# BarisYazici/deep-rl-grasping

Hardware: NVIDIA H100
Metric: SAC grad-steps/sec (batch 256, 64x64 depth) (higher is better)
Workload: dtype bf16x3 (fp32-faithful split, f32 accumulate)

## Files before the change

### deep-rl-grasping_b200/csrc/cg.cu

```cuda
#include <cuda_bf16.h>

#include <cstdio>
#include <cstdlib>

#include "cg.cuh"
#include "common.cuh"
#include "wgmma.cuh"

namespace b2g {
namespace {

constexpr int NMMA_WARPS = 8, NEPI_WARPS = CG_EPI_WARPS, NPROD_WARPS = 2;
constexpr int EPI_WARP0 = NMMA_WARPS, PROD_WARP0 = NMMA_WARPS + NEPI_WARPS;
static_assert(NEPI_WARPS == 4, "the epilogue is one warpgroup: one row of the 128-row tile per lane");
constexpr int NTHREADS = 32 * (PROD_WARP0 + 4);
constexpr int MMA_REGS = 176, EPI_REGS = 136, PROD_REGS = 24;
static_assert(2 * MMA_REGS + EPI_REGS + PROD_REGS <= 512, "register file");
constexpr int STG_BYTES = 2 * 64 * 16 * 4;

__device__ __forceinline__ uint32_t smem_u32(const void* p) { return (uint32_t)__cvta_generic_to_shared(p); }
__device__ __forceinline__ void mbar_init(uint32_t bar, uint32_t count) {
  asm volatile("mbarrier.init.shared::cta.b64 [%0], %1;" ::"r"(bar), "r"(count));
}
__device__ __forceinline__ void mbar_arrive(uint32_t bar) { asm volatile("mbarrier.arrive.shared::cta.b64 _, [%0];" ::"r"(bar) : "memory"); }
__device__ __forceinline__ void mbar_expect_tx(uint32_t bar, uint32_t bytes) {
  asm volatile("mbarrier.arrive.expect_tx.shared::cta.b64 _, [%0], %1;" ::"r"(bar), "r"(bytes) : "memory");
}
__device__ __forceinline__ void mbar_wait(uint32_t bar, uint32_t parity) {
  asm volatile(
      "{\n\t"
      ".reg .pred p;\n\t"
      "CG_WAIT:\n\t"
      "mbarrier.try_wait.parity.shared::cta.b64 p, [%0], %1;\n\t"
      "@p bra CG_DONE;\n\t"
      "bra CG_WAIT;\n\t"
      "CG_DONE:\n\t"
      "}" ::"r"(bar), "r"(parity)
      : "memory");
}
__device__ __forceinline__ bool elect_one() {
  uint32_t pred;
  asm volatile(
      "{\n\t"
      ".reg .pred p;\n\t"
      "elect.sync _|p, 0xffffffff;\n\t"
      "selp.u32 %0, 1, 0, p;\n\t"
      "}"
      : "=r"(pred));
  return pred != 0;
}
__device__ __forceinline__ uint64_t desc_k(uint32_t saddr) { return wg_desc(saddr, 16, 1024); }
__device__ __forceinline__ uint64_t desc_mn(uint32_t saddr, uint32_t lbo) { return wg_desc(saddr, lbo, 1024); }

__device__ __forceinline__ void tma_load(uint32_t dst, const CUtensorMap* map, uint32_t bar, int rank, const int (&c)[5]) {
  switch (rank) {
    case 2:
      asm volatile("cp.async.bulk.tensor.2d.shared::cluster.global.tile.mbarrier::complete_tx::bytes [%0], [%1, {%3, %4}], [%2];" ::"r"(dst), "l"(map),
                   "r"(bar), "r"(c[0]), "r"(c[1])
                   : "memory");
      break;
    case 3:
      asm volatile("cp.async.bulk.tensor.3d.shared::cluster.global.tile.mbarrier::complete_tx::bytes [%0], [%1, {%3, %4, %5}], [%2];" ::"r"(dst),
                   "l"(map), "r"(bar), "r"(c[0]), "r"(c[1]), "r"(c[2])
                   : "memory");
      break;
    case 4:
      asm volatile("cp.async.bulk.tensor.4d.shared::cluster.global.tile.mbarrier::complete_tx::bytes [%0], [%1, {%3, %4, %5, %6}], [%2];" ::"r"(dst),
                   "l"(map), "r"(bar), "r"(c[0]), "r"(c[1]), "r"(c[2]), "r"(c[3])
                   : "memory");
      break;
    default:
      asm volatile("cp.async.bulk.tensor.5d.shared::cluster.global.tile.mbarrier::complete_tx::bytes [%0], [%1, {%3, %4, %5, %6, %7}], [%2];" ::"r"(
                       dst),
                   "l"(map), "r"(bar), "r"(c[0]), "r"(c[1]), "r"(c[2]), "r"(c[3]), "r"(c[4])
                   : "memory");
      break;
  }
}

struct CgPack { CgProblem p[CG_MAX_PROBLEMS]; };
struct Tile { int p, tm, tn, c_begin, c_end; };
struct Walker {
  int p = -1, next_start = 0, tile_start = 0, tiles_n = 1, per = 1, splits = 1, chunks = 0, cps = 0;
  __device__ __forceinline__ bool advance(const CgProblem* __restrict__ probs, int nprob, int tile) {
    bool changed = false;
    while (p < 0 || (p + 1 < nprob && tile >= next_start)) {
      ++p;
      const CgProblem& P = probs[p];
      tile_start = P.tile_start; tiles_n = P.tiles_n; per = P.tiles_m * P.tiles_n; splits = P.splits; chunks = P.chunks;
      cps = (chunks + splits - 1) / splits;
      next_start = p + 1 < nprob ? probs[p + 1].tile_start : 0x7fffffff;
      changed = true;
    }
    return changed;
  }
  __device__ __forceinline__ Tile tile(int t_abs) const {
    int t = t_abs - tile_start, split = 0;
    if (splits > 1) { split = t / per; t -= split * per; }
    Tile ti;
    ti.p = p;
    ti.tm = tiles_n == 1 ? t : t / tiles_n;
    ti.tn = t - ti.tm * tiles_n;
    ti.c_begin = split * cps;
    ti.c_end = min(chunks, ti.c_begin + cps);
    return ti;
  }
};

__device__ __forceinline__ uint32_t pack_bf16x2(float lo, float hi) {
  uint32_t d;
  asm("cvt.rn.bf16x2.f32 %0, %1, %2;" : "=r"(d) : "f"(hi), "f"(lo));
  return d;
}

template <int NT, int NPROD, int TRANS, int KS, int NACC>
__device__ __forceinline__ void mma_chunk(float (&acc)[NACC], uint32_t sbase, uint32_t a_off, uint32_t b_off, uint32_t a_ks, uint32_t b_ks,
                                          uint32_t a_lbo, uint32_t b_lbo, uint32_t a_ps, uint32_t b_ps, uint32_t m_off) {
  constexpr int NPL = NPROD >= 6 ? 3 : (NPROD >= 3 ? 2 : 1), G = NT / 2;
  static_assert(NACC == G * NPL, "one accumulator group of NT columns per product order");
#pragma unroll
  for (int k = 0; k < KS; ++k) {
    uint64_t da[NPL], db[NPL];
#pragma unroll
    for (int pl = 0; pl < NPL; ++pl) {
      const uint32_t pa = sbase + (uint32_t)pl * a_ps + a_off + (uint32_t)k * a_ks + m_off;
      const uint32_t pb = sbase + (uint32_t)pl * b_ps + b_off + (uint32_t)k * b_ks;
      da[pl] = TRANS ? desc_mn(pa, a_lbo) : desc_k(pa);
      db[pl] = TRANS ? desc_mn(pb, b_lbo) : desc_k(pb);
    }
    Wgmma<NT, TRANS>::mma(acc, da[0], db[0]);
    if constexpr (NPL >= 2) Wgmma<NT, TRANS>::mma(acc + G, da[0], db[1]);
    if constexpr (NPL >= 3) Wgmma<NT, TRANS>::mma(acc + 2 * G, da[0], db[2]);
    if constexpr (NPL >= 2) Wgmma<NT, TRANS>::mma(acc + G, da[1], db[0]);
    if constexpr (NPL >= 3) {
      Wgmma<NT, TRANS>::mma(acc + 2 * G, da[1], db[1]);
      Wgmma<NT, TRANS>::mma(acc + 2 * G, da[2], db[0]);
    }
  }
}

__device__ __forceinline__ void mbar_arrive_if(uint32_t bar, bool pred) {
  asm volatile(
      "{\n\t"
      ".reg .pred p;\n\t"
      "setp.ne.u32 p, %1, 0;\n\t"
      "@p mbarrier.arrive.shared::cta.b64 _, [%0];\n\t"
      "}" ::"r"(bar), "r"((uint32_t)pred)
      : "memory");
}
__device__ __forceinline__ void stamp_if(long long* dst, bool pred) {
  asm volatile(
      "{\n\t"
      ".reg .pred p;\n\t"
      ".reg .u64 t;\n\t"
      "mov.u64 t, %%clock64;\n\t"
      "setp.ne.u32 p, %1, 0;\n\t"
      "@p st.global.u64 [%0], t;\n\t"
      "}" ::"l"(dst), "r"((uint32_t)pred)
      : "memory");
}

template <int NT, int NPROD, int TRANS, int KS, class Body>
__device__ __forceinline__ void consume_tile(const CgProblem& P, const Tile& ti, uint32_t ring, uint32_t stg, int slot_bytes, int nstages, uint32_t& s,
                                             uint32_t& ph, uint64_t* bar_full, uint64_t* bar_empty, bool nomma, long long* ctrace, uint32_t& gc,
                                             bool handoff, uint32_t acc_buf, uint32_t& nb, uint64_t* acc_full, uint64_t* acc_empty, Body&& body) {
  constexpr int NGRP = NPROD >= 6 ? 3 : (NPROD >= 3 ? 2 : 1);
  constexpr int NACC = NT / 2 * NGRP;
  const int tid = threadIdx.x, lane = tid & 31, warp = tid >> 5;
  const int wg = warp >> 2, wl = warp & 3, half = wl >> 1;
  float acc[NACC];
#pragma unroll
  for (int j = 0; j < NACC; ++j) acc[j] = 0.f;
  const uint32_t a_ps = (uint32_t)P.a_pstride, b_ps = (uint32_t)P.b_pstride, a_off = P.a_off, b_off = P.b_off, a_ks = P.a_kstep, b_ks = P.b_kstep;
  const uint32_t a_lbo = P.a_lbo, b_lbo = P.b_lbo;
  const uint32_t m_off = TRANS ? (uint32_t)wg * a_lbo : (uint32_t)wg * 8192u;
  uint32_t prev = 0;
  if (nomma) {
    for (int c = ti.c_begin; c < ti.c_end; ++c, ++gc) {
      mbar_wait(smem_u32(&bar_full[s]), (ph >> s) & 1u);
      mbar_arrive_if(smem_u32(&bar_empty[s]), lane == 0);
      ph ^= 1u << s;
      if (++s == (uint32_t)nstages) s = 0;
    }
  } else {
    for (int c = ti.c_begin; c < ti.c_end; ++c, ++gc) {
      long long* const tr = ctrace + gc * 8;
      const bool stamp = ctrace != nullptr && lane == 0 && gc < 64;
      stamp_if(tr + 3, stamp);
      mbar_wait(smem_u32(&bar_full[s]), (ph >> s) & 1u);
      stamp_if(tr + 4, stamp);
      wg_arrive();
      mma_chunk<NT, NPROD, TRANS, KS>(acc, ring + s * (uint32_t)slot_bytes, a_off, b_off, a_ks, b_ks, a_lbo, b_lbo, a_ps, b_ps, m_off);
      wg_commit();
      wg_wait<1>();
      mbar_arrive_if(smem_u32(&bar_empty[prev]), lane == 0 && c > ti.c_begin);
      stamp_if(tr + 5, stamp);
      prev = s;
      ph ^= 1u << s;
      if (++s == (uint32_t)nstages) s = 0;
    }
    wg_wait<0>();
    mbar_arrive_if(smem_u32(&bar_empty[prev]), lane == 0);
  }
  if constexpr (NGRP > 2) {
#pragma unroll
    for (int j = 0; j < NT / 2; ++j) acc[j] = acc[j] + (acc[j + NT / 2] + acc[j + NT]);
  } else if constexpr (NGRP > 1) {
#pragma unroll
    for (int j = 0; j < NT / 2; ++j) acc[j] = acc[j] + acc[j + NT / 2];
  }
  if (handoff) {
    mbar_wait(smem_u32(acc_empty), (nb & 1u) ^ 1u);
    const uint32_t R = 64u * wg + 16u * wl + (uint32_t)(lane >> 2), sw = (uint32_t)(lane >> 2);
    const uint32_t rowa = acc_buf + R * (uint32_t)(NT * 4) + (uint32_t)((lane & 1) * 8);
#pragma unroll
    for (int j = 0; j < NT / 8; ++j)
#pragma unroll
      for (int h = 0; h < 2; ++h) {
        const uint32_t a = rowa + (uint32_t)h * (8u * NT * 4) + ((((uint32_t)(2 * j) + (uint32_t)((lane & 3) >> 1)) ^ sw) << 4);
        asm volatile("st.shared.v2.f32 [%0], {%1,%2};" ::"r"(a), "f"(acc[4 * j + 2 * h]), "f"(acc[4 * j + 2 * h + 1]) : "memory");
      }
    __syncwarp();
    mbar_arrive_if(smem_u32(acc_full), lane == 0);
    ++nb;
    return;
  }
  const int rrow = 32 * (wl & 1) + lane;
  const uint32_t wstg = stg + (uint32_t)wg * 4096u;
#pragma unroll
  for (int R = 0; R < (NT + 63) / 64; ++R) {
    float x[32];
#pragma unroll
    for (int t = 0; t < 4; ++t) {
      const int c0 = 64 * R + 16 * t;
      if (c0 < NT) {
        asm volatile("bar.sync %0, 128;" ::"r"(1 + wg) : "memory");
#pragma unroll
        for (int jj = 0; jj < 2; ++jj)
#pragma unroll
          for (int h = 0; h < 2; ++h) {
            const int row = 16 * wl + (lane >> 2) + 8 * h, chunk = 2 * jj + ((lane & 3) >> 1);
            const int j = c0 / 8 + jj;
            const uint32_t a = wstg + (uint32_t)row * 64u + (uint32_t)((chunk ^ ((row >> 1) & 3)) << 4) + (uint32_t)((lane & 1) * 8);
            asm volatile("st.shared.v2.f32 [%0], {%1,%2};" ::"r"(a), "f"(acc[4 * j + 2 * h]), "f"(acc[4 * j + 2 * h + 1]) : "memory");
          }
        asm volatile("bar.sync %0, 128;" ::"r"(1 + wg) : "memory");
        if (half == (t >> 1)) {
#pragma unroll
          for (int cc = 0; cc < 4; ++cc) {
            const uint32_t a = wstg + (uint32_t)rrow * 64u + (uint32_t)((cc ^ ((rrow >> 1) & 3)) << 4);
            float* xd = x + 16 * (t & 1) + 4 * cc;
            asm volatile("ld.shared.v4.f32 {%0,%1,%2,%3}, [%4];" : "=f"(xd[0]), "=f"(xd[1]), "=f"(xd[2]), "=f"(xd[3]) : "r"(a));
          }
        }
      }
    }
    const int g = 2 * R + half;
    if (32 * g < NT) body(g, x);
  }
}

struct RowOff {
  long long roff = 0, rmoff = 0;
  int ri0 = 0, ri1 = 0;
  __device__ __forceinline__ void set(const CgProblem& Q, int r) {
    const int d0 = Q.d0, d1 = Q.d1;
    const int i0 = r % d0, i12 = r / d0, i1 = i12 % d1, i2 = i12 / d1;
    roff = Q.o_base + (long long)i0 * Q.o0 + (long long)i1 * Q.o1 + (long long)i2 * Q.o2;
    rmoff = Q.m_base + (long long)i0 * Q.m0 + (long long)i1 * Q.m1 + (long long)i2 * Q.m2;
    ri0 = i0; ri1 = i1;
  }
};

__global__ void __launch_bounds__(NTHREADS, 1)
cg_kernel(const __grid_constant__ CgPack pk, int nprob, int total_tiles, const CUtensorMap* __restrict__ maps, int max_stages,
          int dbg, long long* __restrict__ trace) {
  const CgProblem* __restrict__ probs = pk.p;
  extern __shared__ uint8_t smem_raw[];
  __shared__ __align__(8) uint64_t bar_full[CG_MAX_STAGES], bar_empty[CG_MAX_STAGES], acc_full, acc_empty;
  const int tid = threadIdx.x, lane = tid & 31;
  const int warp = __shfl_sync(0xffffffffu, tid >> 5, 0);
  const int trace_cta = dbg >> 8;
  const bool dbg_noload = dbg & 1, dbg_nomma = dbg & 2, dbg_nostore = dbg & 4, dbg_nost = dbg & 16;
  if (tid == 0) {
    for (int s = 0; s < max_stages; ++s) { mbar_init(smem_u32(&bar_full[s]), 1); mbar_init(smem_u32(&bar_empty[s]), NMMA_WARPS); }
    mbar_init(smem_u32(&acc_full), NMMA_WARPS);
    mbar_init(smem_u32(&acc_empty), NEPI_WARPS);
    asm volatile("fence.mbarrier_init.release.cluster;" ::: "memory");
  }
  __syncthreads();
  const uint32_t stg = (smem_u32(smem_raw) + 1023u) & ~1023u;
  const uint32_t ring = stg + STG_BYTES;
  pdl_trigger();
  pdl_wait();

  if (warp >= PROD_WARP0) {
    asm volatile("setmaxnreg.dec.sync.aligned.u32 %0;" ::"n"(PROD_REGS));
    const int pw = warp - PROD_WARP0;
    if (pw >= NPROD_WARPS) return;
    {
      uint32_t gc = 0, s = 0, ph = 0, nbuf = 0;
      int slot_bytes = 0, nstages = 1;
      bool handoff = false;
      Walker w;
      int n2 = 1, nloads = 0, planes = 0, tx = 0;
      const int* tab = nullptr;
      for (int tile = blockIdx.x; tile < total_tiles; tile += gridDim.x) {
        if (w.advance(probs, nprob, tile)) {
          const CgProblem& P = probs[w.p];
          n2 = P.n2; nloads = P.nloads; planes = P.planes; tx = P.tx_bytes; tab = P.tm_tab; handoff = cg_epi_handoff(P.epi);
          if (P.slot_bytes != slot_bytes || P.nstages != nstages) {
            for (int q = 0; q < nstages; ++q) mbar_wait(smem_u32(&bar_empty[q]), ((ph >> q) & 1u) ^ 1u);
            if (nbuf) {
              mbar_wait(smem_u32(&acc_full), (nbuf - 1) & 1u);
              mbar_wait(smem_u32(&acc_empty), (nbuf - 1) & 1u);
              asm volatile("fence.proxy.async.shared::cta;" ::: "memory");
            }
            slot_bytes = P.slot_bytes; nstages = P.nstages; s = 0;
          }
        }
        const Tile ti = w.tile(tile);
        const CgProblem& P = probs[ti.p];
        if (handoff && ti.c_end > ti.c_begin) ++nbuf;
        if (P.dep_ctr) {
          const int* __restrict__ ctr = P.dep_ctr;
          const int x0 = P.dep_by_chunk ? ti.c_begin : ti.tm, x1 = P.dep_by_chunk ? ti.c_end : ti.tm + 1;
          const int lo = x0 * P.dep_rows / P.dep_rows_tile, hi = min(P.dep_tiles - 1, (x1 * P.dep_rows - 1) / P.dep_rows_tile);
          const int expect = P.dep_expect * NEPI_WARPS;
          for (int j = lo + lane; j <= hi; j += 32) {
            int seen;
            do {
              asm volatile("ld.acquire.gpu.global.s32 %0, [%1];" : "=r"(seen) : "l"(ctr + j) : "memory");
              if (seen < expect) __nanosleep(100);
            } while (seen < expect);
          }
          __syncwarp();
          asm volatile("fence.proxy.async.global;" ::: "memory");
        }
        int base[CG_MAX_LOADS][5];
#pragma unroll
        for (int l = 0; l < CG_MAX_LOADS; ++l) {
          if (l < nloads) {
            const CgLoad& L = P.ld[l];
#pragma unroll
            for (int d = 0; d < 5; ++d) base[l][d] = L.c0[d] + ti.tm * L.d_tm[d] + ti.tn * L.d_tn[d];
            if (tab) { base[l][1] += tab[(ti.tm * CG_MAX_LOADS + l) * 2]; base[l][2] += tab[(ti.tm * CG_MAX_LOADS + l) * 2 + 1]; }
          }
        }
        int c1 = n2 > 1 ? ti.c_begin / n2 : 0, c2 = ti.c_begin - c1 * n2;
        for (int c = ti.c_begin; c < ti.c_end; ++c, ++gc) {
          const bool tr = trace && blockIdx.x == trace_cta && pw == 0 && gc < 64 && lane == 0;
          if (tr) trace[gc * 8 + 0] = clock64();
          mbar_wait(smem_u32(&bar_empty[s]), ((ph >> s) & 1u) ^ 1u);
          if (tr) trace[gc * 8 + 1] = clock64();
          const uint32_t full = smem_u32(&bar_full[s]);
          const bool leader = elect_one();
          if (dbg_noload) { if (pw == 0 && leader) mbar_arrive(full); }
          else {
            if (pw == 0 && leader) mbar_expect_tx(full, (uint32_t)tx);
            const uint32_t sbase = ring + s * (uint32_t)slot_bytes;
            int j = 0;
#pragma unroll
            for (int l = 0; l < CG_MAX_LOADS; ++l) {
              if (l < nloads) {
                const CgLoad& L = P.ld[l];
                int crd[5];
#pragma unroll
                for (int d = 0; d < 5; ++d) crd[d] = base[l][d] + c1 * L.d_c1[d] + c2 * L.d_c2[d];
                if (L.plane_box) {
                  if ((j & (NPROD_WARPS - 1)) == pw && leader) tma_load(sbase + (uint32_t)L.smem_off, maps + L.map, full, L.rank, crd);
                  ++j;
                } else {
                  for (int pl = 0; pl < planes; ++pl, ++j) {
#pragma unroll
                    for (int d = 2; d < 5; ++d) if (d == L.rank - 1) crd[d] = pl;
                    if ((j & (NPROD_WARPS - 1)) == pw && leader)
                      tma_load(sbase + (uint32_t)(pl * L.plane_stride + L.smem_off), maps + L.map, full, L.rank, crd);
                  }
                }
              }
            }
          }
          if (tr) { trace[gc * 8 + 2] = clock64(); trace[gc * 8 + 6] = ti.p * 100000 + ti.tm * 10 + ti.tn; }
          if (++c2 == n2) { c2 = 0; ++c1; }
          ph ^= 1u << s;
          if (++s == (uint32_t)nstages) s = 0;
        }
      }
    }
  } else if (warp < NMMA_WARPS) {
    asm volatile("setmaxnreg.inc.sync.aligned.u32 %0;" ::"n"(MMA_REGS));
    const int q = 2 * (warp >> 2) + (warp & 1);
    uint32_t it = 0, s = 0, ph = 0, gc = 0, nb = 0;
    int slot_bytes = 0, nstages = 1;
    Walker w;
    long long* const ctrace = trace && blockIdx.x == trace_cta && warp == 0 ? trace : nullptr;
    const int r = q * 32 + lane;
    int epi = 0, rows_tile = 0, lim_rows = 0, umma_n = 0, n_valid = 0, shape = 0;
    bool handoff = false;
    uint32_t acc_buf = 0;
    long long o_tm = 0;
    RowOff ro;
    for (int tile = blockIdx.x; tile < total_tiles; tile += gridDim.x) {
      if (w.advance(probs, nprob, tile)) {
        const CgProblem& Q = probs[w.p];
        epi = Q.epi; rows_tile = Q.rows_tile; lim_rows = Q.lim_rows; umma_n = Q.umma_n; n_valid = Q.n_valid; o_tm = Q.o_tm;
        ro.set(Q, r);
        shape = cg_shape_key(Q.umma_n, Q.nprod, Q.mn_major != 0, Q.ksteps);
        if (Q.slot_bytes != slot_bytes || Q.nstages != nstages) { slot_bytes = Q.slot_bytes; nstages = Q.nstages; s = 0; }
        handoff = cg_epi_handoff(epi);
        acc_buf = ring + (uint32_t)(nstages * slot_bytes);
      }
      const Tile ti = w.tile(tile);
      if (ti.c_end <= ti.c_begin) continue;
      const CgProblem& P = probs[ti.p];
      const bool valid0 = r < rows_tile && ti.tm * rows_tile + r < lim_rows;
      const long long off0 = ro.roff + (long long)ti.tm * o_tm;
      const int n0 = ti.tn * umma_n;
      const bool tre = trace && blockIdx.x == trace_cta && warp == 0 && lane == 0 && it < 16;
      if (tre) trace[512 + it * 4 + 0] = clock64();
      auto body = [&](int g, float (&x)[32]) {
        const int ng = n0 + 32 * g;
        if (dbg_nostore || ng >= n_valid || !valid0) return;
        float* dst = P.out_f + off0 + (long long)(ng >> 5) * P.f_grp;
        if (epi == CG_EPI_RAW) {
          if (P.atomic) {
#pragma unroll
            for (int j = 0; j < 8; ++j)
              asm volatile("red.global.add.v4.f32 [%0], {%1,%2,%3,%4};" ::"l"(dst + 4 * j), "f"(x[4 * j]), "f"(x[4 * j + 1]), "f"(x[4 * j + 2]),
                           "f"(x[4 * j + 3])
                           : "memory");
          } else {
#pragma unroll
            for (int j = 0; j < 8; ++j) *reinterpret_cast<float4*>(dst + 4 * j) = make_float4(x[4 * j], x[4 * j + 1], x[4 * j + 2], x[4 * j + 3]);
          }
          return;
        }
        const float sc = P.scale;
        if (P.atomic) {
#pragma unroll
          for (int j = 0; j < 8; ++j)
            asm volatile("red.global.add.v4.f32 [%0], {%1,%2,%3,%4};" ::"l"(dst + 4 * j), "f"(x[4 * j] * sc), "f"(x[4 * j + 1] * sc),
                         "f"(x[4 * j + 2] * sc), "f"(x[4 * j + 3] * sc)
                         : "memory");
        } else {
#pragma unroll
          for (int j = 0; j < 8; ++j)
            *reinterpret_cast<float4*>(dst + 4 * j) = make_float4(x[4 * j] * sc, x[4 * j + 1] * sc, x[4 * j + 2] * sc, x[4 * j + 3] * sc);
          if (P.dp_n > 1) {
            const int i4 = (int)((dst - P.dp_gbase) >> 2), per4 = P.dp_per4;
#pragma unroll
            for (int j = 0; j < 8; ++j) {
              const int owner = (i4 + j) / per4;
              if (owner != P.dp_rank)
                reinterpret_cast<float4*>(P.dp_recv[owner])[(size_t)P.dp_rank * per4 + (i4 + j - owner * per4)] =
                    make_float4(x[4 * j] * sc, x[4 * j + 1] * sc, x[4 * j + 2] * sc, x[4 * j + 3] * sc);
            }
          }
        }
      };
#define CG_CONSUME(NT, NPROD, TRANS, KS)                                                                                                      \
  consume_tile<NT, NPROD, TRANS, KS>(P, ti, ring, stg, slot_bytes, nstages, s, ph, bar_full, bar_empty, dbg_nomma, ctrace, gc, handoff, acc_buf, \
                                     nb, &acc_full, &acc_empty, body)
      switch (shape) {
        case cg_shape_key(32, 6, false, 4): CG_CONSUME(32, 6, 0, 4); break;
        case cg_shape_key(64, 6, false, 4): CG_CONSUME(64, 6, 0, 4); break;
        case cg_shape_key(64, 3, false, 4): CG_CONSUME(64, 3, 0, 4); break;
        case cg_shape_key(128, 3, false, 4): CG_CONSUME(128, 3, 0, 4); break;
        case cg_shape_key(64, 3, true, 4): CG_CONSUME(64, 3, 1, 4); break;
        case cg_shape_key(64, 3, true, 9): CG_CONSUME(64, 3, 1, 9); break;
        case cg_shape_key(128, 3, true, 4): CG_CONSUME(128, 3, 1, 4); break;
        default: __trap();
      }
#undef CG_CONSUME
      if (tre) {
        trace[512 + it * 4 + 1] = clock64();
        trace[512 + it * 4 + 2] = handoff;
        trace[512 + it * 4 + 3] = ti.p * 100000 + ti.tm * 10 + ti.tn;
      }
      ++it;
    }
  } else {
    asm volatile("setmaxnreg.inc.sync.aligned.u32 %0;" ::"n"(EPI_REGS));
    const int ew = warp - EPI_WARP0;
    const int r = ew * 32 + lane;
    uint32_t ne = 0;
    int slot_bytes = 0, nstages = 1;
    Walker w;
    int epi = 0, rows_tile = 0, lim_rows = 0, umma_n = 0, out_planes = 0, grp_stride = 32, n_valid = 0, grp_tab = 0;
    bool handoff = false;
    uint32_t acc_buf = 0;
    long long o_tm = 0, m_tm = 0;
    RowOff ro;
    const float* __restrict__ bias = nullptr;
    const uint16_t* __restrict__ mask = nullptr;
    for (int tile = blockIdx.x; tile < total_tiles; tile += gridDim.x) {
      if (w.advance(probs, nprob, tile)) {
        const CgProblem& Q = probs[w.p];
        epi = Q.epi; rows_tile = Q.rows_tile; lim_rows = Q.lim_rows; umma_n = Q.umma_n; out_planes = Q.out_planes;
        grp_stride = Q.grp_stride; n_valid = Q.n_valid; o_tm = Q.o_tm; m_tm = Q.m_tm; bias = Q.bias; mask = Q.mask; grp_tab = Q.grp_tab;
        ro.set(Q, r);
        if (Q.slot_bytes != slot_bytes || Q.nstages != nstages) { slot_bytes = Q.slot_bytes; nstages = Q.nstages; }
        handoff = cg_epi_handoff(epi);
        acc_buf = ring + (uint32_t)(nstages * slot_bytes);
      }
      const Tile ti = w.tile(tile);
      if (ti.c_end <= ti.c_begin || !handoff) continue;
      const CgProblem& P = probs[ti.p];
      const bool valid0 = r < rows_tile && ti.tm * rows_tile + r < lim_rows;
      const long long off0 = ro.roff + (long long)ti.tm * o_tm, moff0 = ro.rmoff + (long long)ti.tm * m_tm;
      const int n0 = ti.tn * umma_n, ngroups = umma_n >> 5;
      auto group_at = [&](int g, bool& valid, long long& off, long long& moff) {
        const int ng = n0 + 32 * g;
        valid = valid0; off = off0; moff = moff0;
        if (grp_tab) {
          const int gg = ng >> 5;
          valid = valid0 && ro.ri0 < P.grp_lim0[gg] && ro.ri1 < P.grp_lim1[gg];
          off = off0 + P.grp_off[gg]; moff = moff0 + P.grp_moff[gg] - ng;
        }
      };
      const bool tre = trace && blockIdx.x == trace_cta && ew == 0 && lane == 0 && ne < 16;
      if (tre) trace[576 + ne * 4 + 0] = clock64();
      uint32_t mbits[4] = {0u, 0u, 0u, 0u};
      if (epi == CG_EPI_DGRAD && !dbg_nostore) {
#pragma unroll
        for (int g = 0; g < 4; ++g) {
          bool valid;
          long long off, moff;
          group_at(g, valid, off, moff);
          const int ng = n0 + 32 * g;
          if (g < ngroups && valid && ng < n_valid) {
            uint4 mk[4];
#pragma unroll
            for (int j = 0; j < 4; ++j) mk[j] = __ldg(reinterpret_cast<const uint4*>(mask + moff + ng) + j);
#pragma unroll
            for (int j = 0; j < 4; ++j) {
              const uint32_t wd[4] = {mk[j].x, mk[j].y, mk[j].z, mk[j].w};
#pragma unroll
              for (int uu = 0; uu < 4; ++uu) {
                if (wd[uu] & 0x00007FFFu) mbits[g] |= 1u << (8 * j + 2 * uu);
                if (wd[uu] & 0x7FFF0000u) mbits[g] |= 1u << (8 * j + 2 * uu + 1);
              }
            }
          }
        }
      }
      mbar_wait(smem_u32(&acc_full), ne & 1u);
      if (tre) trace[576 + ne * 4 + 1] = clock64();
      const bool split_fin = P.ws != nullptr;
      float* __restrict__ wsrow = split_fin ? P.ws + ((size_t)(ti.tm * w.tiles_n + ti.tn) * 128 + r) * umma_n : nullptr;
      auto body = [&](int g, float (&x)[32], int pass) {
        const int ng = n0 + 32 * g;
        bool valid;
        long long off, moff;
        group_at(g, valid, off, moff);
        if (pass == 0 && split_fin) {
#pragma unroll
          for (int j = 0; j < 8; ++j)
            asm volatile("red.global.add.v4.f32 [%0], {%1,%2,%3,%4};" ::"l"(wsrow + 32 * g + 4 * j), "f"(x[4 * j]), "f"(x[4 * j + 1]), "f"(x[4 * j + 2]),
                         "f"(x[4 * j + 3])
                         : "memory");
          return;
        }
        const bool live = !dbg_nostore && ng < n_valid;
        float4 bv[8];
        if (epi == CG_EPI_ACT && live) {
#pragma unroll
          for (int j = 0; j < 8; ++j) bv[j] = __ldg(reinterpret_cast<const float4*>(bias + (long long)(ng >> 5) * P.bias_grp) + j);
        }
        if (!live) return;
        if (epi == CG_EPI_ACT) {
#pragma unroll
          for (int j = 0; j < 8; ++j) {
            x[4 * j] = fmaxf(x[4 * j] + bv[j].x, 0.f); x[4 * j + 1] = fmaxf(x[4 * j + 1] + bv[j].y, 0.f);
            x[4 * j + 2] = fmaxf(x[4 * j + 2] + bv[j].z, 0.f); x[4 * j + 3] = fmaxf(x[4 * j + 3] + bv[j].w, 0.f);
          }
          if (P.f0 > 0 && valid && !dbg_nost) {
            float* dst = P.out_f + (long long)ti.tm * P.f_tm + (long long)r * P.f0 + (long long)(ng >> 5) * P.f_grp;
#pragma unroll
            for (int j = 0; j < 8; ++j) *reinterpret_cast<float4*>(dst + 4 * j) = make_float4(x[4 * j], x[4 * j + 1], x[4 * j + 2], x[4 * j + 3]);
          }
        } else {
          const uint32_t mb = g == 0 ? mbits[0] : g == 1 ? mbits[1] : g == 2 ? mbits[2] : mbits[3];
#pragma unroll
          for (int j = 0; j < 32; ++j)
            if (!((mb >> j) & 1u)) x[j] = 0.f;
          if (P.colsum) {
            float cs[32];
#pragma unroll
            for (int j = 0; j < 32; ++j) cs[j] = x[j];
#pragma unroll
            for (int wd = 16; wd >= 1; wd >>= 1) {
              const bool up = (lane & wd) != 0;
#pragma unroll
              for (int j = 0; j < wd; ++j) {
                const float send = up ? cs[j] : cs[j + wd], keep = up ? cs[j + wd] : cs[j];
                cs[j] = keep + __shfl_xor_sync(0xffffffffu, send, wd);
              }
            }
            atomicAdd(P.colsum + ((ng + lane) & P.colsum_mask), cs[0]);
          }
        }
        const long long gcol = grp_tab ? 0 : (long long)(ng >> 5) * grp_stride;
#pragma unroll 1
        for (int pl = 0; pl < out_planes; ++pl) {
          uint32_t pk[16];
#pragma unroll
          for (int j = 0; j < 16; ++j) {
            pk[j] = pack_bf16x2(x[2 * j], x[2 * j + 1]);
            x[2 * j] -= __uint_as_float(pk[j] << 16);
            x[2 * j + 1] -= __uint_as_float(pk[j] & 0xFFFF0000u);
          }
          if (valid && !dbg_nost) {
            uint16_t* dst = P.out_p[pl] + off + gcol;
#pragma unroll
            for (int j = 0; j < 4; ++j) *reinterpret_cast<uint4*>(dst + 8 * j) = make_uint4(pk[4 * j], pk[4 * j + 1], pk[4 * j + 2], pk[4 * j + 3]);
          }
        }
      };
      const uint32_t rowa = acc_buf + (uint32_t)(r * umma_n * 4), sw = (uint32_t)(r & 7);
      for (int g = 0; g < ngroups; ++g) {
        float x[32];
#pragma unroll
        for (int cc = 0; cc < 8; ++cc) {
          const uint32_t a = rowa + ((((uint32_t)(8 * g + cc)) ^ sw) << 4);
          asm volatile("ld.shared.v4.f32 {%0,%1,%2,%3}, [%4];" : "=f"(x[4 * cc]), "=f"(x[4 * cc + 1]), "=f"(x[4 * cc + 2]), "=f"(x[4 * cc + 3]) : "r"(a));
        }
        if (g == ngroups - 1) {
          __syncwarp();
          mbar_arrive_if(smem_u32(&acc_empty), lane == 0);
        }
        body(g, x, 0);
      }
      ++ne;
      bool last_arriver = !split_fin;
      if (split_fin) {
        __syncwarp();
        int old = 0;
        if (lane == 0) { __threadfence(); old = atomicAdd(P.ws_cnt + (ti.tm * w.tiles_n + ti.tn) * NEPI_WARPS + ew, 1); }
        old = __shfl_sync(0xffffffffu, old, 0);
        last_arriver = old == w.splits - 1;
        if (last_arriver) {
          __threadfence();
          if (lane == 0) P.ws_cnt[(ti.tm * w.tiles_n + ti.tn) * NEPI_WARPS + ew] = 0;
          for (int g = 0; g < ngroups; ++g) {
            float x[32];
#pragma unroll
            for (int j = 0; j < 8; ++j) {
              const float4 sum = __ldcg(reinterpret_cast<const float4*>(wsrow + 32 * g) + j);
              x[4 * j] = sum.x; x[4 * j + 1] = sum.y; x[4 * j + 2] = sum.z; x[4 * j + 3] = sum.w;
              __stcg(reinterpret_cast<float4*>(wsrow + 32 * g) + j, make_float4(0.f, 0.f, 0.f, 0.f));
            }
            body(g, x, 1);
          }
        }
      }
      __syncwarp();
      if (lane == 0 && P.done_ctr && last_arriver) {
        __threadfence();
        atomicAdd(P.done_ctr + ti.tm, 1);
      }
      if (tre) { trace[576 + (ne - 1) * 4 + 2] = clock64(); trace[576 + (ne - 1) * 4 + 3] = ti.p * 100000 + ti.tm * 10 + ti.tn; }
    }
  }
}

typedef CUresult (*EncodeTiledFn)(CUtensorMap*, CUtensorMapDataType, cuuint32_t, void*, const cuuint64_t*, const cuuint64_t*, const cuuint32_t*,
                                  const cuuint32_t*, CUtensorMapInterleave, CUtensorMapSwizzle, CUtensorMapL2promotion, CUtensorMapFloatOOBfill);
EncodeTiledFn g_encode = nullptr;

}

bool cg_shape_supported(int umma_n, int nprod, bool mn_major, int ksteps) {
  switch (cg_shape_key(umma_n, nprod, mn_major, ksteps)) {
    case cg_shape_key(32, 6, false, 4): case cg_shape_key(64, 6, false, 4): case cg_shape_key(64, 3, false, 4): case cg_shape_key(128, 3, false, 4):
    case cg_shape_key(64, 3, true, 4): case cg_shape_key(64, 3, true, 9): case cg_shape_key(128, 3, true, 4): return true;
    default: return false;
  }
}

int cg_smem_limit() { return 226 * 1024 - STG_BYTES; }

int cg_encode_map(CUtensorMap* out, const void* base, int rank, const uint64_t* dims, const uint64_t* strides_bytes, const uint32_t* box,
                  const uint32_t* elem_strides) {
  if (!g_encode) {
    cudaDriverEntryPointQueryResult q;
    void* fn = nullptr;
    if (cudaGetDriverEntryPoint("cuTensorMapEncodeTiled", &fn, cudaEnableDefault, &q) != cudaSuccess || !fn || q != cudaDriverEntryPointSuccess) return -1;
    g_encode = (EncodeTiledFn)fn;
  }
  cuuint64_t gd[5], gs[5];
  cuuint32_t bx[5], es[5];
  for (int i = 0; i < rank; ++i) { gd[i] = dims[i]; bx[i] = box[i]; es[i] = elem_strides ? elem_strides[i] : 1; }
  for (int i = 0; i + 1 < rank; ++i) gs[i] = strides_bytes[i];
  const CUresult r = g_encode(out, CU_TENSOR_MAP_DATA_TYPE_BFLOAT16, (cuuint32_t)rank, const_cast<void*>(base), gd, gs, bx, es, CU_TENSOR_MAP_INTERLEAVE_NONE,
                              CU_TENSOR_MAP_SWIZZLE_128B, CU_TENSOR_MAP_L2_PROMOTION_L2_256B, CU_TENSOR_MAP_FLOAT_OOB_FILL_NONE);
  return r == CUDA_SUCCESS ? 0 : (int)r;
}

int cg_finalize(CgGroup& g, int smem_budget) {
  int start = 0, slot = 0;
  g.flops = 0;
  for (int i = 0; i < g.n; ++i) {
    CgProblem& P = g.host[i];
    P.tile_start = start;
    start += P.tiles_m * P.tiles_n * P.splits;
    for (int l = 0; l < P.nloads; ++l) {
      CgLoad& L = P.ld[l];
      L.plane_stride = L.smem_off >= P.b_off ? P.b_pstride : P.a_pstride;
      if (L.plane_box && L.box_bytes != L.plane_stride) return -2;
    }
    const int need = P.b_off + P.planes * P.b_pstride;
    P.slot_bytes = (need + 1023) / 1024 * 1024;
    slot = slot > P.slot_bytes ? slot : P.slot_bytes;
  }
  g.total_tiles = start;
  const int avail = smem_budget - 1024 ;
  g.slot_bytes = slot; g.nstages = 0;
  int ring = 0;
  for (int i = 0; i < g.n; ++i) {
    CgProblem& P = g.host[i];
    const int acc = cg_epi_handoff(P.epi) ? cg_acc_bytes(P.umma_n) : 0;
    const int avail_ring = avail - acc;
    P.nstages = P.slot_bytes > 0 ? avail_ring / P.slot_bytes : 0;
    if (P.nstages > CG_MAX_STAGES) P.nstages = CG_MAX_STAGES;
    if (P.nstages < 2) return -1;
    P.slot_bytes = avail_ring / P.nstages / 1024 * 1024;
    g.nstages = g.nstages > P.nstages ? g.nstages : P.nstages;
    ring = ring > P.nstages * P.slot_bytes + acc ? ring : P.nstages * P.slot_bytes + acc;
  }
  g.ring_bytes = ring;
  return 0;
}

long long* g_cg_trace = nullptr;

cudaError_t cg_launch(const CgGroup& g, const CUtensorMap* dev_maps, int num_sms, cudaStream_t s, bool pdl, int debug_flags) {
  if (g.total_tiles <= 0 || (debug_flags & 8)) return cudaSuccess;
  static bool attr_set = false;
  if (!attr_set) {
    cudaError_t e = cudaFuncSetAttribute(cg_kernel, cudaFuncAttributeMaxDynamicSharedMemorySize, 226 * 1024);
    if (e != cudaSuccess) return e;
    attr_set = true;
  }
  const int smem = 1024 + STG_BYTES + g.ring_bytes;
  const int grid = g.total_tiles < num_sms ? g.total_tiles : num_sms;
  CgPack pk;
  static_assert(sizeof(CgPack) < 28 * 1024, "problem list must fit the kernel parameter space (32,764 B)");
  for (int i = 0; i < g.n; ++i) pk.p[i] = g.host[i];
  cudaError_t e = launch_pdl(cg_kernel, dim3(grid), dim3(NTHREADS), (size_t)smem, s, pdl, pk, g.n, g.total_tiles, dev_maps, g.nstages, debug_flags, g_cg_trace);
  if (e != cudaSuccess) fprintf(stderr, "cg_launch %s: %s (grid %d, %d threads, smem %d)\n", g.name, cudaGetErrorString(e), grid, NTHREADS, smem);
  return e;
}

}
```

### deep-rl-grasping_b200/csrc/cg.cuh

```cuda
#pragma once
#include <cuda.h>
#include <cuda_runtime.h>
#include <stdint.h>

namespace b2g {

constexpr int CG_MAX_LOADS = 4;
constexpr int CG_MAX_PROBLEMS = 16;
constexpr int CG_MAX_STAGES = 8;
constexpr int CG_MAX_PLANES = 3;
constexpr int CG_EPI_WARPS = 4;

enum CgEpiKind : int {
  CG_EPI_ACT = 0,
  CG_EPI_RAW = 1,
  CG_EPI_DGRAD = 2,
  CG_EPI_WGRAD = 3,
};
__host__ __device__ constexpr bool cg_epi_handoff(int epi) { return epi == CG_EPI_ACT || epi == CG_EPI_DGRAD; }
__host__ __device__ constexpr int cg_acc_bytes(int umma_n) { return 128 * umma_n * 4; }

struct CgLoad {
  int map;
  int rank;
  int box_bytes;
  int smem_off;
  int plane_stride;
  int plane_box;
  int c0[5];
  int d_tm[5], d_tn[5], d_c1[5], d_c2[5];
};

struct CgProblem {
  int tile_start, tiles_m, tiles_n, splits;
  int chunks, n2;
  int nloads, planes;
  int a_pstride, b_pstride;
  int tx_bytes;
  int slot_bytes, nstages;
  CgLoad ld[CG_MAX_LOADS];
  const int* tm_tab;
  int mn_major;
  int ksteps;
  int a_off, b_off;
  int a_kstep, b_kstep;
  int a_lbo, b_lbo;
  int umma_n;
  int nprod;
  int epi;
  int rows_tile;
  int lim_rows;
  int d0, d1;
  long long o_tm; int o0, o1, o2; long long o_base;
  long long m_tm; int m0, m1, m2; long long m_base;
  int n_valid;
  int grp_stride;
  int grp_tab;
  int grp_off[8], grp_moff[8], grp_lim0[8], grp_lim1[8];
  int out_planes;
  uint16_t* out_p[CG_MAX_PLANES];
  float* out_f;
  long long f_tm; int f0;
  const float* bias;
  int bias_grp;
  long long f_grp;
  const uint16_t* mask;
  float* colsum;
  int colsum_mask;
  int atomic;
  float scale;
  int* done_ctr;
  const int* dep_ctr;
  int dep_rows, dep_rows_tile, dep_tiles, dep_expect;
  float* ws;
  int* ws_cnt;
  float* dp_recv[8];
  const float* dp_gbase;
  int dp_rank, dp_n, dp_per4;
  int dep_by_chunk;
};

struct CgGroup {
  CgProblem host[CG_MAX_PROBLEMS];
  int n = 0;
  int total_tiles = 0;
  int slot_bytes = 0, nstages = 0, ring_bytes = 0;
  const char* name = "";
  double flops = 0;
};

int cg_encode_map(CUtensorMap* out, const void* base, int rank, const uint64_t* dims, const uint64_t* strides_bytes, const uint32_t* box,
                  const uint32_t* elem_strides);
int cg_finalize(CgGroup& g, int smem_budget);
cudaError_t cg_launch(const CgGroup& g, const CUtensorMap* dev_maps, int num_sms, cudaStream_t s, bool pdl, int debug_flags);
int cg_smem_limit();
__host__ __device__ constexpr int cg_shape_key(int umma_n, int nprod, bool mn_major, int ksteps) {
  return ksteps * 8192 + umma_n * 16 + nprod * 2 + (mn_major ? 1 : 0);
}
bool cg_shape_supported(int umma_n, int nprod, bool mn_major, int ksteps);

}
```

### deep-rl-grasping_b200/csrc/engine_v2.cu

```cuda
#include <cuda_bf16.h>

#include <algorithm>
#include <cstdio>
#include <cstdlib>
#include <cstring>

#include "sac_internal.cuh"

namespace b2g {
namespace {

struct Gather2Args {
  GatherArgs g;
  uint16_t* a1[2][3];
  uint16_t* fp[3][3];
  int KF, Ci, OH, OW;
};

__device__ __forceinline__ void split3(float y, uint16_t& p0, uint16_t& p1, uint16_t& p2) {
  const __nv_bfloat16 h0 = __float2bfloat16_rn(y);
  const float r1 = y - __bfloat162float(h0);
  const __nv_bfloat16 h1 = __float2bfloat16_rn(r1);
  const float r2 = r1 - __bfloat162float(h1);
  p0 = __bfloat16_as_ushort(h0); p1 = __bfloat16_as_ushort(h1); p2 = __bfloat16_as_ushort(__float2bfloat16_rn(r2));
}

__global__ void __launch_bounds__(512) gather2_kernel(Gather2Args a) {
  extern __shared__ uint16_t sm_planes[];
  const GatherArgs& g = a.g;
  const int b = blockIdx.x, which = blockIdx.y, tid = threadIdx.x;
  const int Ci = a.Ci, HW = g.H * g.W, npx = HW * Ci;
  const int Ec = npx + 4;
  long long slot = b;
  if (g.indices) slot = g.indices[b];
  else if (g.rng_counters) {
    slot = philox_slot(g.seed, (unsigned long long)g.rng_counters[4], b, (unsigned long long)g.rng_counters[5]);
    if (g.ring_cap > 0) slot = ring_slot(g.rng_counters[6], (int)slot, g.ring_cap);
    if (g.indices_out && which == 0 && tid == 0) g.indices_out[b] = (int)slot;
  }
  const unsigned char* __restrict__ src =
      g.obs_frame ? g.frames + (size_t)(which ? g.next_frame : g.obs_frame)[slot] * g.frame_bytes
                  : reinterpret_cast<const unsigned char*>((which ? g.next_obs : g.obs) + (size_t)slot * Ec);
  const double clip_obs = g.normc[1];
  const bool norm_obs = g.normc[3] != 0.0;
  const float scale = g.scale;
  const int rowe = g.W * Ci, pitch = rowe + 8, plane_e = g.H * pitch;
  for (int e4 = tid; e4 < (npx >> 2); e4 += blockDim.x) {
    const float4 v = frame_load4(src, g.fmt, npx, Ci, 4 * e4);
    float y[4] = {v.x, v.y, v.z, v.w};
    if (norm_obs) {
      const double2 m0 = *reinterpret_cast<const double2*>(g.mean + 4 * e4), m1 = *reinterpret_cast<const double2*>(g.mean + 4 * e4 + 2);
      const double2 i0 = *reinterpret_cast<const double2*>(g.var + 4 * e4), i1 = *reinterpret_cast<const double2*>(g.var + 4 * e4 + 2);
      y[0] = (float)fmin(fmax(((double)y[0] - m0.x) * i0.x, -clip_obs), clip_obs);
      y[1] = (float)fmin(fmax(((double)y[1] - m0.y) * i0.y, -clip_obs), clip_obs);
      y[2] = (float)fmin(fmax(((double)y[2] - m1.x) * i1.x, -clip_obs), clip_obs);
      y[3] = (float)fmin(fmax(((double)y[3] - m1.y) * i1.y, -clip_obs), clip_obs);
    }
    uint16_t p[3][4];
#pragma unroll
    for (int j = 0; j < 4; ++j) split3(y[j] / scale, p[0][j], p[1][j], p[2][j]);
#pragma unroll
    for (int pl = 0; pl < 3; ++pl) {
      const uint2 w = make_uint2((uint32_t)p[pl][0] | ((uint32_t)p[pl][1] << 16), (uint32_t)p[pl][2] | ((uint32_t)p[pl][3] << 16));
      const int e = 4 * e4, row = e / rowe, col = e - row * rowe;
      *reinterpret_cast<uint2*>(sm_planes + pl * plane_e + row * pitch + col) = w;
    }
  }
  if (tid == 0) {
    float yy = frame_elem(src, g.fmt, npx, Ci, npx);
    if (norm_obs) yy = (float)fmin(fmax(((double)yy - g.mean[npx]) * g.var[npx], -clip_obs), clip_obs);
    yy = yy / scale;
    uint16_t p0, p1, p2;
    split3(yy, p0, p1, p2);
    const size_t fo = (size_t)b * g.FS + g.feat_col, po = (size_t)b * a.KF + g.feat_col;
    if (which) { g.F_t[fo] = yy; a.fp[2][0][po] = p0; a.fp[2][1][po] = p1; a.fp[2][2][po] = p2; }
    else {
      g.F_pi[fo] = yy; g.F_v[fo] = yy;
      a.fp[0][0][po] = p0; a.fp[0][1][po] = p1; a.fp[0][2][po] = p2;
      a.fp[1][0][po] = p0; a.fp[1][1][po] = p1; a.fp[1][2][po] = p2;
    }
  }
  __syncthreads();
  const int seg = 8 * Ci;
  const int K1 = 64 * Ci, nruns = a.OH * a.OW * 8;
  const size_t img = (size_t)b * a.OH * a.OW * K1;
  for (int i = tid; i < nruns * (seg / 8); i += blockDim.x) {
    const int part = i % (seg / 8), run = i / (seg / 8);
    const int ky = run & 7, patch = run >> 3;
    const int oy = patch / a.OW, ox = patch - oy * a.OW;
    const int so = (4 * oy + ky) * pitch + 4 * ox * Ci + 8 * part;
    const size_t go = img + (size_t)patch * K1 + ky * seg + 8 * part;
#pragma unroll
    for (int pl = 0; pl < 3; ++pl) {
      const uint16_t* sp = sm_planes + pl * plane_e + so;
      const uint2 lo = *reinterpret_cast<const uint2*>(sp), hi = *reinterpret_cast<const uint2*>(sp + 4);
      *reinterpret_cast<uint4*>(a.a1[which][pl] + go) = make_uint4(lo.x, lo.y, hi.x, hi.y);
    }
  }
  if (which == 0 && g.act) {
    const int feat_dim = g.feat_col + 1;
    if (tid < g.n_act) {
      const float av = g.act[slot * g.n_act + tid];
      g.F_v[(size_t)b * g.FS + feat_dim + tid] = av;
      uint16_t p0, p1, p2;
      split3(av, p0, p1, p2);
      const size_t po = (size_t)b * a.KF + feat_dim + tid;
      a.fp[1][0][po] = p0; a.fp[1][1][po] = p1; a.fp[1][2][po] = p2;
    }
    if (tid == 32) {
      float r = g.rew[slot];
      if (g.normc[4] != 0.0) r = (float)fmin(fmax((double)r * g.normc[0], -g.normc[2]), g.normc[2]);
      g.rew_out[b] = r;
      g.done_out[b] = g.done[slot];
    }
  }
}

struct Plane2Job {
  const float* src;
  uint16_t* dst[3];
  int R, N, np;
  int transpose;
  int ld, off0;
  int tile_start;
};

__global__ void __launch_bounds__(256) planes2_kernel(const Plane2Job* __restrict__ jobs, const int* __restrict__ cta_job) {
  __shared__ float tile[64][33];
  const Plane2Job job = jobs[cta_job[blockIdx.x]];
  const int t = blockIdx.x - job.tile_start;
  const int tiles_n = (job.N + 31) / 32;
  const int r0 = (t / tiles_n) * 64, n0 = (t % tiles_n) * 32;
  const int tid = threadIdx.x;
  const bool vec_ok = (job.N & 3) == 0;
  for (int i = tid; i < 64 * 8; i += 256) {
    const int rr = i >> 3, c4 = i & 7, r = r0 + rr, n = n0 + 4 * c4;
    float4 v = make_float4(0.f, 0.f, 0.f, 0.f);
    if (r < job.R) {
      const float* sp = job.src + (size_t)r * job.N + n;
      if (vec_ok && n + 3 < job.N) v = *reinterpret_cast<const float4*>(sp);
      else { if (n < job.N) v.x = sp[0]; if (n + 1 < job.N) v.y = sp[1]; if (n + 2 < job.N) v.z = sp[2]; if (n + 3 < job.N) v.w = sp[3]; }
    }
    tile[rr][4 * c4] = v.x; tile[rr][4 * c4 + 1] = v.y; tile[rr][4 * c4 + 2] = v.z; tile[rr][4 * c4 + 3] = v.w;
    if (!job.transpose && r < job.R) {
      const float x[4] = {v.x, v.y, v.z, v.w};
      uint16_t p[3][4];
#pragma unroll
      for (int u = 0; u < 4; ++u) split3(x[u], p[0][u], p[1][u], p[2][u]);
      for (int k = 0; k < job.np; ++k) {
        uint16_t* d = job.dst[k] + (size_t)r * job.ld + job.off0 + n;
        if (n + 3 < job.N && (((size_t)r * job.ld + job.off0 + n) & 3) == 0)
          *reinterpret_cast<uint2*>(d) = make_uint2((uint32_t)p[k][0] | ((uint32_t)p[k][1] << 16), (uint32_t)p[k][2] | ((uint32_t)p[k][3] << 16));
        else
          for (int u = 0; u < 4; ++u) if (n + u < job.N) d[u] = p[k][u];
      }
    }
  }
  if (!job.transpose) return;
  __syncthreads();
  {
    const int nn = tid >> 3, g8 = tid & 7, n = n0 + nn, rb = r0 + 8 * g8;
    if (n < job.N && rb < job.R) {
      uint16_t p[3][8];
#pragma unroll
      for (int u = 0; u < 8; ++u) split3(tile[8 * g8 + u][nn], p[0][u], p[1][u], p[2][u]);
      const size_t o = (size_t)(n + job.off0) * job.ld + rb;
      for (int k = 0; k < job.np; ++k) {
        uint16_t* d = job.dst[k] + o;
        if (rb + 7 < job.R && (o & 7) == 0)
          *reinterpret_cast<uint4*>(d) = make_uint4((uint32_t)p[k][0] | ((uint32_t)p[k][1] << 16), (uint32_t)p[k][2] | ((uint32_t)p[k][3] << 16),
                                                    (uint32_t)p[k][4] | ((uint32_t)p[k][5] << 16), (uint32_t)p[k][6] | ((uint32_t)p[k][7] << 16));
        else
          for (int u = 0; u < 8; ++u) if (rb + u < job.R) d[u] = p[k][u];
      }
    }
  }
}

int add_maps(V2State& v, uint16_t* const* planes, int np, int rank, std::initializer_list<uint64_t> dims, std::initializer_list<uint64_t> strides_b,
             std::initializer_list<uint32_t> box, std::initializer_list<uint32_t> estr = {}, bool allow_whole = true) {
  uint64_t d[5] = {1, 1, 1, 1, 1}, s[5] = {0, 0, 0, 0, 0};
  uint32_t bx[5] = {1, 1, 1, 1, 1}, es[5] = {1, 1, 1, 1, 1};
  int i = 0; for (auto x : dims) d[i++] = x;
  i = 0; for (auto x : strides_b) s[i++] = x;
  i = 0; for (auto x : box) bx[i++] = x;
  i = 0; for (auto x : estr) es[i++] = x;
  if (rank >= 5 || np < 1) return -1;
  size_t rows = 1;
  for (int k = 1; k < rank; ++k) rows *= (bx[k] + es[k] - 1) / es[k];
  const size_t box_bytes = rows * bx[0] * 2;
  const bool whole = allow_whole && np > 1 && box_bytes % 1024 == 0;
  const long long pitch = np > 1 ? (long long)((const char*)planes[1] - (const char*)planes[0]) : 16;
  for (int p = 2; p < np; ++p)
    if ((const char*)planes[p] - (const char*)planes[p - 1] != pitch) return -1;
  if (pitch <= 0 || pitch % 16) return -1;
  d[rank] = (uint64_t)np; s[rank - 1] = (uint64_t)pitch; bx[rank] = whole ? (uint32_t)np : 1u; es[rank] = 1;
  CUtensorMap m;
  if (cg_encode_map(&m, planes[0], rank + 1, d, s, bx, es) != 0) return -1;
  v.maps.push_back(m);
  v.map_whole.push_back(whole ? 1 : 0);
  v.map_box_bytes.push_back((int)box_bytes);
  return (int)v.maps.size() - 1;
}

const V2State* g_mk_state = nullptr;
CgLoad mk_load(int map, int rank, int smem_off) {
  CgLoad L;
  memset(&L, 0, sizeof(L));
  L.map = map; L.rank = rank + 1; L.smem_off = smem_off;
  L.plane_box = g_mk_state->map_whole[map];
  L.box_bytes = g_mk_state->map_box_bytes[map];
  return L;
}

CgProblem kmajor(int planes, int n_tile, int chunks, int n2, int a_box_rows) {
  CgProblem P;
  memset(&P, 0, sizeof(P));
  P.tiles_m = P.tiles_n = P.splits = 1;
  P.chunks = chunks; P.n2 = n2;
  P.planes = planes;
  P.a_off = 0; P.a_pstride = 128 * 128;
  P.b_off = planes * P.a_pstride; P.b_pstride = n_tile * 128;
  P.tx_bytes = planes * (a_box_rows * 128 + n_tile * 128);
  P.mn_major = 0; P.ksteps = 4; P.a_kstep = P.b_kstep = 32;
  P.umma_n = n_tile;
  P.nprod = planes == 3 ? 6 : (planes == 2 ? 3 : 1);
  P.d0 = 1 << 20; P.d1 = 1;
  P.grp_stride = 32; P.f_grp = 32; P.bias_grp = 32;
  P.scale = 1.f;
  return P;
}

CgProblem mnmajor(int planes, int kr, int a_atoms, int b_atoms, int chunks) {
  CgProblem P;
  memset(&P, 0, sizeof(P));
  P.tiles_m = P.tiles_n = P.splits = 1;
  P.chunks = chunks; P.n2 = chunks > 0 ? chunks : 1;
  P.planes = planes;
  const int atom = kr * 128;
  P.a_off = 0; P.a_pstride = atom;
  P.b_off = 2 * planes * atom; P.b_pstride = b_atoms * atom;
  P.tx_bytes = planes * (a_atoms + b_atoms) * atom;
  P.mn_major = 1; P.ksteps = kr / 16; P.a_kstep = P.b_kstep = 2048;
  P.a_lbo = planes * atom; P.b_lbo = atom;
  P.umma_n = 64 * b_atoms;
  P.nprod = planes == 3 ? 6 : (planes == 2 ? 3 : 1);
  P.d0 = 1 << 20; P.d1 = 1;
  P.grp_stride = 32; P.f_grp = 32; P.bias_grp = 32;
  P.scale = 1.f;
  P.epi = CG_EPI_WGRAD; P.rows_tile = 128;
  return P;
}

int push_group(b2g_sac* h, std::vector<CgGroup>& list, CgGroup& g, const char* name) {
  g.name = name;
  if (cg_finalize(g, cg_smem_limit()) != 0) return b2g_fail(B2G_EINVAL, std::string("engine v2: stage ring of group ") + name + " does not fit shared memory");
  for (int i = 0; i < g.n; ++i) {
    const CgProblem& P = g.host[i];
    if (P.planes * P.umma_n > 256) return b2g_fail(B2G_EINVAL, std::string("engine v2: planes x tile width exceeds one accumulator buffer (group ") + name + ")");
    if (!cg_shape_supported(P.umma_n, P.nprod, P.mn_major != 0, P.ksteps))
      return b2g_fail(B2G_EINVAL, std::string("engine v2: no cg_kernel instance for the tile shape of a problem in group ") + name);
    g.flops += 2.0 * P.tiles_m * 128.0 * P.tiles_n * P.umma_n * P.chunks * 64.0;
  }
  list.push_back(g);
  return 0;
}

struct Wire { int cons, ci, prod, pi, dep_rows, dep_rows_tile, by_chunk; };
int fuse_groups(b2g_sac* h, const std::vector<const CgGroup*>& parts, const std::vector<Wire>& wires, const char* name, std::vector<CgGroup>& out, int& n_ctr) {
  CgGroup f;
  std::vector<int> first(parts.size());
  for (size_t gi = 0; gi < parts.size(); ++gi) {
    first[gi] = f.n;
    for (int i = 0; i < parts[gi]->n; ++i) {
      if (f.n >= CG_MAX_PROBLEMS) return b2g_fail(B2G_EINVAL, std::string("engine v2: too many problems in fused launch ") + name);
      f.host[f.n++] = parts[gi]->host[i];
    }
  }
  std::vector<int> ctr_of(f.n, -1);
  for (const Wire& w : wires) {
    const int pi = first[w.prod] + w.pi, qi = first[w.cons] + w.ci;
    CgProblem& Pp = f.host[pi];
    CgProblem& Pc = f.host[qi];
    if (!cg_epi_handoff(Pp.epi))
      return b2g_fail(B2G_EINVAL, std::string("engine v2: a wired producer must have an ACT or DGRAD epilogue (fused launch ") + name + ")");
    if (Pc.dep_ctr && ctr_of[pi] < 0) {
      ctr_of[pi] = (int)(intptr_t)Pc.dep_ctr - 1;
      Pc.dep_expect += Pp.ws ? Pp.tiles_n : Pp.tiles_n * Pp.splits;
      continue;
    }
    if (Pp.splits > 1 && (Pp.splits - 1) * ((Pp.chunks + Pp.splits - 1) / Pp.splits) >= Pp.chunks)
      return b2g_fail(B2G_EINVAL, std::string("engine v2: a wired split-K producer has an empty split (fused launch ") + name + ")");
    if (ctr_of[pi] < 0) { ctr_of[pi] = n_ctr; n_ctr += Pp.tiles_m; }
    Pc.dep_rows = w.dep_rows; Pc.dep_rows_tile = w.dep_rows_tile; Pc.dep_tiles = Pp.tiles_m; Pc.dep_by_chunk = w.by_chunk;
    Pc.dep_expect = Pp.ws ? Pp.tiles_n : Pp.tiles_n * Pp.splits;
    Pc.dep_ctr = (const int*)(intptr_t)(ctr_of[pi] + 1);
  }
  for (int i = 0; i < f.n; ++i) f.host[i].done_ctr = (int*)(intptr_t)(ctr_of[i] + 1);
  return push_group(h, out, f, name);
}

void bind_counters(std::vector<CgGroup>& groups, int* base) {
  for (CgGroup& g : groups)
    for (int i = 0; i < g.n; ++i) {
      CgProblem& P = g.host[i];
      const intptr_t d = (intptr_t)P.done_ctr, c = (intptr_t)P.dep_ctr;
      P.done_ctr = d ? base + (d - 1) : nullptr;
      P.dep_ctr = c ? base + (c - 1) : nullptr;
    }
}

int check_split(const char* var, int chunks, int splits) {
  auto empty = [chunks](int s) { return (s - 1) * ((chunks + s - 1) / s) >= chunks; };
  if (!empty(splits)) return 0;
  std::string ok;
  for (int s = 1; s <= chunks; ++s)
    if (!empty(s)) ok += (ok.empty() ? "" : ", ") + std::to_string(s);
  return b2g_fail(B2G_EINVAL, std::string(var) + "=" + std::to_string(splits) + " leaves a K-split of " + std::to_string(chunks) +
                                  " chunks empty; use one of " + ok);
}

}

int v2_alloc(b2g_sac* h) {
  V2State& v = h->v2;
  const int B = h->B, Ci = h->Cimg, K1 = 64 * Ci, KF = v.KF;
  const size_t n1 = (size_t)B * 225 * 32, n2 = (size_t)B * 36 * 64, n3 = (size_t)B * 1024, na = (size_t)B * 225 * K1, nf = (size_t)B * KF;
  uint16_t *bH1, *bH2, *bH3, *bF, *bA1;
  if (int rc = dev_alloc(h->allocs, h->stream, &bH1, 9 * n1)) return rc;
  if (int rc = dev_alloc(h->allocs, h->stream, &bH2, 9 * n2)) return rc;
  if (int rc = dev_alloc(h->allocs, h->stream, &bH3, 9 * n3)) return rc;
  if (int rc = dev_alloc(h->allocs, h->stream, &bF, 9 * nf)) return rc;
  if (int rc = dev_alloc(h->allocs, h->stream, &bA1, 6 * na)) return rc;
  for (int n = 0; n < 3; ++n)
    for (int p = 0; p < 3; ++p) {
      v.H1[n][p] = bH1 + (n * 3 + p) * n1; v.H2[n][p] = bH2 + (n * 3 + p) * n2; v.H3[n][p] = bH3 + (n * 3 + p) * n3;
      v.F[n][p] = bF + (n * 3 + p) * nf;
    }
  for (int w = 0; w < 2; ++w) for (int p = 0; p < 3; ++p) v.A1[w][p] = bA1 + (w * 3 + p) * na;
  if (int rc = dev_alloc(h->allocs, h->stream, &v.z0v, (size_t)B * 3 * h->H)) return rc;
  auto palloc = [&](uint16_t** arr, int np, size_t count) -> int {
    const size_t pitch = (count + 63) / 64 * 64;
    uint16_t* base = nullptr;
    if (int rc = dev_alloc(h->allocs, h->stream, &base, pitch * np)) return rc;
    for (int p = 0; p < np; ++p) arr[p] = base + p * pitch;
    return 0;
  };
  if (int rc = palloc(v.dz0pi, 2, (size_t)B * h->H)) return rc;
  if (int rc = palloc(v.dz0v, 2, (size_t)B * 3 * h->H)) return rc;
  if (int rc = palloc(v.dZ1, 2, (size_t)B * 225 * 64)) return rc;
  for (int n = 0; n < 2; ++n) {
    if (int rc = palloc(v.dZ4[n], 2, (size_t)B * 512)) return rc;
    if (int rc = palloc(v.dZ3[n], 2, n3)) return rc;
    if (int rc = palloc(v.dZ2[n], 2, n2)) return rc;
    if (int rc = palloc(v.W2n[n], 2, 512 * 64)) return rc;
    if (int rc = palloc(v.W3n[n], 2, 576 * 64)) return rc;
    if (int rc = palloc(v.Wfn[n], 2, 1024 * 512)) return rc;
    if (int rc = palloc(v.K0n[n], 2, (size_t)KF * (n == 1 ? 3 : 1) * h->H)) return rc;
  }
  if (int rc = palloc(v.W1T[0], 3, (size_t)64 * K1)) return rc;
  if (int rc = palloc(v.W1T[1], 3, (size_t)32 * K1)) return rc;
  for (int n = 0; n < 3; ++n) {
    if (int rc = palloc(v.W2T[n], 3, 64 * 512)) return rc;
    if (int rc = palloc(v.W3T[n], 3, 64 * 576)) return rc;
    if (int rc = palloc(v.WfT[n], 3, 512 * 1024)) return rc;
    if (int rc = palloc(v.K0T[n], 3, (size_t)(n == 1 ? 3 : 1) * h->H * KF)) return rc;
  }
  return 0;
}

int v2_create(b2g_sac* h) {
  V2State& v = h->v2;
  g_mk_state = &v;
  const int B = h->B, Ci = h->Cimg, K1 = 64 * Ci, KF = v.KF, FS = h->FS, H = h->H;
  const size_t n1 = (size_t)B * 225 * 32;
  const char* nets[3] = {"model/pi", "model/values_fn", "target/values_fn"};
  std::vector<Plane2Job> jobs;
  int start = 0;
  auto add_job = [&](const float* src, int R, int N, uint16_t* const* dst, int np, int transpose, int ld, int off0) {
    Plane2Job j{};
    j.src = src; j.R = R; j.N = N; j.np = np; j.transpose = transpose; j.ld = ld; j.off0 = off0; j.tile_start = start;
    for (int k = 0; k < np; ++k) j.dst[k] = dst[k];
    start += ((R + 63) / 64) * ((N + 31) / 32);
    jobs.push_back(j);
  };
  add_job(h->p("model/pi/cnn1/w"), K1, 32, v.W1T[0], 3, 1, K1, 0);
  add_job(h->p("model/values_fn/cnn1/w"), K1, 32, v.W1T[0], 3, 1, K1, 32);
  add_job(h->p("target/values_fn/cnn1/w"), K1, 32, v.W1T[1], 3, 1, K1, 0);
  for (int n = 0; n < 3; ++n) {
    add_job(h->p(std::string(nets[n]) + "/cnn2/w"), 512, 64, v.W2T[n], 3, 1, 512, 0);
    add_job(h->p(std::string(nets[n]) + "/cnn3/w"), 576, 64, v.W3T[n], 3, 1, 576, 0);
    add_job(h->p(std::string(nets[n]) + "/cnn_fc1/w"), 1024, 512, v.WfT[n], 3, 1, 1024, 0);
  }
  add_job(h->p("model/pi/fc0/kernel"), h->feat_dim, H, v.K0T[0], 3, 1, KF, 0);
  add_job(h->p("model/values_fn/vf/fc0/kernel"), h->feat_dim, H, v.K0T[1], 3, 1, KF, 0);
  add_job(h->p("model/values_fn/qf1/fc0/kernel"), h->feat_dim + h->A, H, v.K0T[1], 3, 1, KF, H);
  add_job(h->p("model/values_fn/qf2/fc0/kernel"), h->feat_dim + h->A, H, v.K0T[1], 3, 1, KF, 2 * H);
  add_job(h->p("target/values_fn/vf/fc0/kernel"), h->feat_dim, H, v.K0T[2], 3, 1, KF, 0);
  for (int n = 0; n < 2; ++n) {
    add_job(h->p(std::string(nets[n]) + "/cnn2/w"), 512, 64, v.W2n[n], 2, 0, 64, 0);
    add_job(h->p(std::string(nets[n]) + "/cnn3/w"), 576, 64, v.W3n[n], 2, 0, 64, 0);
    add_job(h->p(std::string(nets[n]) + "/cnn_fc1/w"), 1024, 512, v.Wfn[n], 2, 0, 512, 0);
  }
  add_job(h->p("model/pi/fc0/kernel"), h->feat_dim, H, v.K0n[0], 2, 0, H, 0);
  add_job(h->p("model/values_fn/vf/fc0/kernel"), h->feat_dim, H, v.K0n[1], 2, 0, 3 * H, 0);
  add_job(h->p("model/values_fn/qf1/fc0/kernel"), h->feat_dim + h->A, H, v.K0n[1], 2, 0, 3 * H, H);
  add_job(h->p("model/values_fn/qf2/fc0/kernel"), h->feat_dim + h->A, H, v.K0n[1], 2, 0, 3 * H, 2 * H);
  v.n_plane_jobs = (int)jobs.size();
  v.plane_ctas = start;
  Plane2Job* dj = nullptr;
  if (int rc = dev_alloc(h->allocs, h->stream, &dj, jobs.size())) return rc;
  CK(cudaMemcpyAsync(dj, jobs.data(), jobs.size() * sizeof(Plane2Job), cudaMemcpyHostToDevice, h->stream));
  CK(cudaStreamSynchronize(h->stream));
  v.plane_jobs = dj;
  {
    std::vector<int> cj((size_t)start);
    for (size_t k = 0; k < jobs.size(); ++k)
      for (int t = jobs[k].tile_start; t < (k + 1 < jobs.size() ? jobs[k + 1].tile_start : start); ++t) cj[t] = (int)k;
    if (int rc = upload_table(h->allocs, h->stream, cj, &v.plane_cta_job)) return rc;
  }

  { const char* e = getenv("B2G_SPLIT_FC1"); v.split_fc1 = e ? std::max(1, atoi(e)) : 3; }
  { const char* e = getenv("B2G_SPLIT_FC1_DGRAD"); v.split_fc1_dgrad = e ? std::max(1, atoi(e)) : 1; }
  const int NP = 3;
  const long long h1_net = (long long)3 * n1;
  {
    CgGroup g;
    for (int w = 0; w < 2; ++w) {
      const int N = w == 0 ? 64 : 32;
      const int mA = add_maps(v, v.A1[w], NP, 2, {(uint64_t)K1, (uint64_t)B * 225}, {(uint64_t)K1 * 2}, {64, 128});
      const int mB = add_maps(v, v.W1T[w], NP, 2, {(uint64_t)K1, (uint64_t)N}, {(uint64_t)K1 * 2}, {64, (uint32_t)N});
      if (mA < 0 || mB < 0) return b2g_fail(B2G_ECUDA, "engine v2: cuTensorMapEncodeTiled failed (conv1)");
      CgProblem P = kmajor(NP, N, Ci, Ci, 128);
      P.nloads = 2;
      P.ld[0] = mk_load(mA, 2, 0); P.ld[0].d_tm[1] = 128; P.ld[0].d_c2[0] = 64;
      P.ld[1] = mk_load(mB, 2, P.b_off); P.ld[1].d_c2[0] = 64;
      P.tiles_m = (B * 225 + 127) / 128;
      P.epi = CG_EPI_ACT; P.rows_tile = 128; P.lim_rows = B * 225;
      P.o_tm = 128 * 32; P.o0 = 32; P.n_valid = N; P.out_planes = 3;
      P.grp_stride = (int)h1_net;
      const int net0 = w == 0 ? 0 : 2;
      for (int p = 0; p < 3; ++p) P.out_p[p] = v.H1[net0][p];
      P.bias = h->p(std::string(nets[net0]) + "/cnn1/b");
      P.bias_grp = w == 0 ? (int)(h->p("model/values_fn/cnn1/b") - h->p("model/pi/cnn1/b")) : 32;
      g.host[g.n++] = P;
    }
    if (int rc = push_group(h, v.fwd, g, "conv1_fwd")) return rc;
  }
  {
    CgGroup g;
    for (int n = 0; n < 3; ++n) {
      const int mA = add_maps(v, v.H1[n], NP, 4, {64, 14, 15, (uint64_t)B}, {64, 15 * 64, 225 * 64}, {64, 12, 12, 3}, {1, 2, 2, 1});
      const int mB = add_maps(v, v.W2T[n], NP, 2, {512, 64}, {1024}, {64, 64});
      if (mA < 0 || mB < 0) return b2g_fail(B2G_ECUDA, "engine v2: cuTensorMapEncodeTiled failed (conv2)");
      CgProblem P = kmajor(NP, 64, 8, 2, 108);
      P.nloads = 2;
      P.ld[0] = mk_load(mA, 4, 0); P.ld[0].d_tm[3] = 3; P.ld[0].d_c1[2] = 1; P.ld[0].d_c2[1] = 2;
      P.ld[1] = mk_load(mB, 2, P.b_off); P.ld[1].d_c1[0] = 128; P.ld[1].d_c2[0] = 64;
      P.tiles_m = (B + 2) / 3;
      P.epi = CG_EPI_ACT; P.rows_tile = 108; P.lim_rows = B * 36;
      P.o_tm = 108 * 64; P.o0 = 64; P.n_valid = 64; P.out_planes = 3;
      for (int p = 0; p < 3; ++p) P.out_p[p] = v.H2[n][p];
      P.bias = h->p(std::string(nets[n]) + "/cnn2/b"); P.bias_grp = 32;
      g.host[g.n++] = P;
    }
    if (int rc = push_group(h, v.fwd, g, "conv2_fwd")) return rc;
  }
  {
    CgGroup g;
    for (int n = 0; n < 3; ++n) {
      const int mA = add_maps(v, v.H2[n], NP, 4, {64, 6, 6, (uint64_t)B}, {128, 6 * 128, 36 * 128}, {64, 4, 4, 8});
      const int mB = add_maps(v, v.W3T[n], NP, 2, {576, 64}, {1152}, {64, 64});
      if (mA < 0 || mB < 0) return b2g_fail(B2G_ECUDA, "engine v2: cuTensorMapEncodeTiled failed (conv3)");
      CgProblem P = kmajor(NP, 64, 9, 3, 128);
      P.nloads = 2;
      P.ld[0] = mk_load(mA, 4, 0); P.ld[0].d_tm[3] = 8; P.ld[0].d_c1[2] = 1; P.ld[0].d_c2[1] = 1;
      P.ld[1] = mk_load(mB, 2, P.b_off); P.ld[1].d_c1[0] = 192; P.ld[1].d_c2[0] = 64;
      P.tiles_m = (B + 7) / 8;
      P.epi = CG_EPI_ACT; P.rows_tile = 128; P.lim_rows = B * 16;
      P.o_tm = 128 * 64; P.o0 = 64; P.n_valid = 64; P.out_planes = 3;
      for (int p = 0; p < 3; ++p) P.out_p[p] = v.H3[n][p];
      P.bias = h->p(std::string(nets[n]) + "/cnn3/b"); P.bias_grp = 32;
      g.host[g.n++] = P;
    }
    if (int rc = push_group(h, v.fwd, g, "conv3_fwd")) return rc;
  }
  {
    CgGroup g;
    for (int n = 0; n < 3; ++n) {
      const int mA = add_maps(v, v.H3[n], NP, 2, {1024, (uint64_t)B}, {2048}, {64, 128});
      const int mB = add_maps(v, v.WfT[n], NP, 2, {1024, 512}, {2048}, {64, 64});
      if (mA < 0 || mB < 0) return b2g_fail(B2G_ECUDA, "engine v2: cuTensorMapEncodeTiled failed (cnn_fc1)");
      CgProblem P = kmajor(NP, 64, 16, 16, 128);
      P.nloads = 2;
      P.ld[0] = mk_load(mA, 2, 0); P.ld[0].d_tm[1] = 128; P.ld[0].d_c2[0] = 64;
      P.ld[1] = mk_load(mB, 2, P.b_off); P.ld[1].d_tn[1] = 64; P.ld[1].d_c2[0] = 64;
      P.tiles_m = (B + 127) / 128; P.tiles_n = 8;
      P.epi = CG_EPI_ACT; P.rows_tile = 128; P.lim_rows = B;
      P.o_tm = (long long)128 * KF; P.o0 = KF; P.n_valid = 512; P.out_planes = 3;
      for (int p = 0; p < 3; ++p) P.out_p[p] = v.F[n][p];
      P.bias = h->p(std::string(nets[n]) + "/cnn_fc1/b"); P.bias_grp = 32;
      P.out_f = h->F[n]; P.f_tm = (long long)128 * FS; P.f0 = FS; P.f_grp = 32;
      if (v.split_fc1 > 1) {
        P.splits = v.split_fc1;
        if (int rc = check_split("B2G_SPLIT_FC1", P.chunks, P.splits)) return rc;
        if (int rc = dev_alloc(h->allocs, h->stream, &P.ws, (size_t)P.tiles_m * P.tiles_n * 128 * 64)) return rc;
        if (int rc = dev_alloc(h->allocs, h->stream, &P.ws_cnt, (size_t)P.tiles_m * P.tiles_n * CG_EPI_WARPS)) return rc;
      }
      g.host[g.n++] = P;
    }
    if (int rc = push_group(h, v.fwd, g, "fc1_fwd")) return rc;
  }
  {
    CgGroup g;
    float* z0out[3] = {h->z0[0], v.z0v, h->z0[4]};
    for (int n = 0; n < 3; ++n) {
      const int Nn = n == 1 ? 3 * H : H;
      const int mA = add_maps(v, v.F[n], NP, 2, {(uint64_t)KF, (uint64_t)B}, {(uint64_t)KF * 2}, {64, 128});
      const int mB = add_maps(v, v.K0T[n], NP, 2, {(uint64_t)KF, (uint64_t)Nn}, {(uint64_t)KF * 2}, {64, 64});
      if (mA < 0 || mB < 0) return b2g_fail(B2G_ECUDA, "engine v2: cuTensorMapEncodeTiled failed (fc0)");
      CgProblem P = kmajor(NP, 64, KF / 64, KF / 64, 128);
      P.nloads = 2;
      P.ld[0] = mk_load(mA, 2, 0); P.ld[0].d_tm[1] = 128; P.ld[0].d_c2[0] = 64;
      P.ld[1] = mk_load(mB, 2, P.b_off); P.ld[1].d_tn[1] = 64; P.ld[1].d_c2[0] = 64;
      P.tiles_m = (B + 127) / 128; P.tiles_n = Nn / 64;
      P.epi = CG_EPI_RAW; P.rows_tile = 128; P.lim_rows = B;
      P.o_tm = (long long)128 * Nn; P.o0 = Nn; P.n_valid = Nn;
      P.splits = P.chunks; P.atomic = 1;
      P.out_f = z0out[n];
      g.host[g.n++] = P;
    }
    if (int rc = push_group(h, v.fwd, g, "heads_fc0")) return rc;
  }

  const int NB = 2;
  {
    CgGroup g;
    for (int n = 0; n < 2; ++n) {
      const int Kd = n == 0 ? H : 3 * H;
      uint16_t* const* dz = n == 0 ? v.dz0pi : v.dz0v;
      const int mA = add_maps(v, dz, NB, 2, {(uint64_t)Kd, (uint64_t)B}, {(uint64_t)Kd * 2}, {64, 128});
      const int mB = add_maps(v, v.K0n[n], NB, 2, {(uint64_t)Kd, (uint64_t)KF}, {(uint64_t)Kd * 2}, {64, 128});
      if (mA < 0 || mB < 0) return b2g_fail(B2G_ECUDA, "engine v2: cuTensorMapEncodeTiled failed (heads dgrad)");
      CgProblem P = kmajor(NB, 128, Kd / 64, Kd / 64, 128);
      P.nloads = 2;
      P.ld[0] = mk_load(mA, 2, 0); P.ld[0].d_tm[1] = 128; P.ld[0].d_c2[0] = 64;
      P.ld[1] = mk_load(mB, 2, P.b_off); P.ld[1].d_tn[1] = 128; P.ld[1].d_c2[0] = 64;
      P.tiles_m = (B + 127) / 128; P.tiles_n = 4;
      P.epi = CG_EPI_DGRAD; P.rows_tile = 128; P.lim_rows = B;
      P.o_tm = 128 * 512; P.o0 = 512; P.n_valid = 512; P.out_planes = 2;
      for (int p = 0; p < 2; ++p) P.out_p[p] = v.dZ4[n][p];
      P.mask = v.F[n][0]; P.m_tm = (long long)128 * KF; P.m0 = KF;
      P.colsum = h->g(std::string(nets[n]) + "/cnn_fc1/b"); P.colsum_mask = 511;
      g.host[g.n++] = P;
    }
    if (int rc = push_group(h, v.bwd_groups, g, "heads_dgrad")) return rc;
  }
  {
    CgGroup g;
    for (int n = 0; n < 2; ++n) {
      {
        const int mA = add_maps(v, v.dZ4[n], NB, 2, {512, (uint64_t)B}, {1024}, {64, 128});
        const int mB = add_maps(v, v.Wfn[n], NB, 2, {512, 1024}, {1024}, {64, 128});
        if (mA < 0 || mB < 0) return b2g_fail(B2G_ECUDA, "engine v2: cuTensorMapEncodeTiled failed (fc1 dgrad)");
        CgProblem P = kmajor(NB, 128, 8, 8, 128);
        P.nloads = 2;
        P.ld[0] = mk_load(mA, 2, 0); P.ld[0].d_tm[1] = 128; P.ld[0].d_c2[0] = 64;
        P.ld[1] = mk_load(mB, 2, P.b_off); P.ld[1].d_tn[1] = 128; P.ld[1].d_c2[0] = 64;
        P.tiles_m = (B + 127) / 128; P.tiles_n = 8;
        P.epi = CG_EPI_DGRAD; P.rows_tile = 128; P.lim_rows = B;
        P.o_tm = 128 * 1024; P.o0 = 1024; P.n_valid = 1024; P.out_planes = 2;
        for (int p = 0; p < 2; ++p) P.out_p[p] = v.dZ3[n][p];
        P.mask = v.H3[n][0]; P.m_tm = 128 * 1024; P.m0 = 1024;
        P.colsum = h->g(std::string(nets[n]) + "/cnn3/b"); P.colsum_mask = 63;
        if (v.split_fc1_dgrad > 1) {
          P.splits = v.split_fc1_dgrad;
          if (int rc = check_split("B2G_SPLIT_FC1_DGRAD", P.chunks, P.splits)) return rc;
          if (int rc = dev_alloc(h->allocs, h->stream, &P.ws, (size_t)P.tiles_m * P.tiles_n * 128 * 128)) return rc;
          if (int rc = dev_alloc(h->allocs, h->stream, &P.ws_cnt, (size_t)P.tiles_m * P.tiles_n * CG_EPI_WARPS)) return rc;
        }
        g.host[g.n++] = P;
      }
      {
        const int mA = add_maps(v, v.H3[n], NB, 2, {1024, (uint64_t)B}, {2048}, {64, 64});
        const int mB = add_maps(v, v.dZ4[n], NB, 2, {512, (uint64_t)B}, {1024}, {64, 64}, {}, false);
        if (mA < 0 || mB < 0) return b2g_fail(B2G_ECUDA, "engine v2: cuTensorMapEncodeTiled failed (fc1 wgrad)");
        CgProblem P = mnmajor(NB, 64, 2, 2, (B + 63) / 64);
        P.nloads = 4;
        for (int a = 0; a < 2; ++a) {
          P.ld[a] = mk_load(mA, 2, a * P.a_lbo); P.ld[a].c0[0] = 64 * a; P.ld[a].d_tm[0] = 128; P.ld[a].d_c2[1] = 64;
          P.ld[2 + a] = mk_load(mB, 2, P.b_off + a * 8192); P.ld[2 + a].c0[0] = 64 * a; P.ld[2 + a].d_tn[0] = 128; P.ld[2 + a].d_c2[1] = 64;
        }
        P.tiles_m = 8; P.tiles_n = 4;
        P.lim_rows = 1024; P.o_tm = 128 * 512; P.o0 = 512; P.n_valid = 512;
        P.out_f = h->g(std::string(nets[n]) + "/cnn_fc1/w"); P.atomic = 0;
        g.host[g.n++] = P;
      }
    }
    if (int rc = push_group(h, v.bwd_groups, g, "fc1_bwd")) return rc;
  }
  {
    CgGroup g;
    std::vector<int> tab(5 * CG_MAX_LOADS * 2, 0);
    for (int tm = 0; tm < 5; ++tm)
      for (int a = 0; a < 2; ++a) {
        const int pos = 2 * tm + a;
        tab[(tm * CG_MAX_LOADS + a) * 2] = pos % 3; tab[(tm * CG_MAX_LOADS + a) * 2 + 1] = pos / 3;
      }
    const int* dtab = nullptr;
    if (int rc = upload_table(h->allocs, h->stream, tab, &dtab)) return rc;
    for (int n = 0; n < 2; ++n) {
      {
        const int mA = add_maps(v, v.dZ3[n], NB, 4, {64, 4, 4, (uint64_t)B}, {128, 512, 2048}, {64, 6, 6, 3});
        const int mB = add_maps(v, v.W3n[n], NB, 2, {64, 576}, {128}, {64, 64});
        if (mA < 0 || mB < 0) return b2g_fail(B2G_ECUDA, "engine v2: cuTensorMapEncodeTiled failed (conv3 dgrad)");
        CgProblem P = kmajor(NB, 64, 9, 3, 108);
        P.nloads = 2;
        P.ld[0] = mk_load(mA, 4, 0); P.ld[0].d_tm[3] = 3; P.ld[0].d_c1[2] = -1; P.ld[0].d_c2[1] = -1;
        P.ld[1] = mk_load(mB, 2, P.b_off); P.ld[1].d_c1[1] = 192; P.ld[1].d_c2[1] = 64;
        P.tiles_m = (B + 2) / 3;
        P.epi = CG_EPI_DGRAD; P.rows_tile = 108; P.lim_rows = B * 36;
        P.o_tm = 108 * 64; P.o0 = 64; P.n_valid = 64; P.out_planes = 2;
        for (int p = 0; p < 2; ++p) P.out_p[p] = v.dZ2[n][p];
        P.mask = v.H2[n][0]; P.m_tm = 108 * 64; P.m0 = 64;
        P.colsum = h->g(std::string(nets[n]) + "/cnn2/b"); P.colsum_mask = 63;
        g.host[g.n++] = P;
      }
      {
        const int mA = add_maps(v, v.H2[n], NB, 4, {64, 6, 6, (uint64_t)B}, {128, 768, 4608}, {64, 4, 4, 4});
        const int mB = add_maps(v, v.dZ3[n], NB, 2, {64, (uint64_t)B * 16}, {128}, {64, 64});
        if (mA < 0 || mB < 0) return b2g_fail(B2G_ECUDA, "engine v2: cuTensorMapEncodeTiled failed (conv3 wgrad)");
        CgProblem P = mnmajor(NB, 64, 2, 1, (B + 3) / 4);
        P.nloads = 3;
        for (int a = 0; a < 2; ++a) { P.ld[a] = mk_load(mA, 4, a * P.a_lbo); P.ld[a].d_c2[3] = 4; }
        P.ld[2] = mk_load(mB, 2, P.b_off); P.ld[2].d_c2[1] = 64;
        P.tm_tab = dtab;
        P.tiles_m = 5; P.tiles_n = 1;
        P.splits = std::max(1, std::min(P.chunks, std::max(14, (P.chunks + 15) / 16)));
        P.lim_rows = 576; P.o_tm = 128 * 64; P.o0 = 64; P.n_valid = 64;
        P.out_f = h->g(std::string(nets[n]) + "/cnn3/w"); P.atomic = 1;
        g.host[g.n++] = P;
      }
    }
    if (int rc = push_group(h, v.bwd_groups, g, "conv3_bwd")) return rc;
  }
  {
    CgGroup g;
    for (int n = 0; n < 2; ++n) {
      const int mA = add_maps(v, v.dZ2[n], NB, 4, {64, 6, 6, (uint64_t)B}, {128, 768, 4608}, {64, 8, 8, 2});
      const int mB = add_maps(v, v.W2n[n], NB, 2, {64, 512}, {128}, {64, 64}, {}, false);
      if (mA < 0 || mB < 0) return b2g_fail(B2G_ECUDA, "engine v2: cuTensorMapEncodeTiled failed (conv2 dgrad)");
      CgProblem P = kmajor(NB, 128, 4, 2, 128);
      P.tx_bytes = NB * (128 * 128 + 2 * 64 * 128);
      P.nloads = 3;
      P.ld[0] = mk_load(mA, 4, 0); P.ld[0].d_tm[3] = 2; P.ld[0].d_c1[2] = -1; P.ld[0].d_c2[1] = -1;
      for (int py = 0; py < 2; ++py) {
        P.ld[1 + py] = mk_load(mB, 2, P.b_off + py * 64 * 128);
        P.ld[1 + py].c0[1] = py * 128; P.ld[1 + py].d_c1[1] = 256; P.ld[1 + py].d_c2[1] = 64;
      }
      P.tiles_m = (B + 1) / 2;
      P.epi = CG_EPI_DGRAD; P.rows_tile = 128; P.lim_rows = B * 64;
      P.d0 = 8; P.d1 = 8;
      P.o_tm = 2 * 225 * 64; P.o0 = 2 * 64; P.o1 = 2 * 15 * 64; P.o2 = 225 * 64; P.o_base = n * 32;
      P.m_tm = 2 * 225 * 32; P.m0 = 2 * 32; P.m1 = 2 * 15 * 32; P.m2 = 225 * 32; P.m_base = 0;
      P.grp_tab = 1;
      for (int py = 0; py < 2; ++py)
        for (int px = 0; px < 2; ++px) {
          const int gg = py * 2 + px;
          P.grp_off[gg] = (py * 15 + px) * 64; P.grp_moff[gg] = (py * 15 + px) * 32;
          P.grp_lim0[gg] = (15 - px + 1) / 2; P.grp_lim1[gg] = (15 - py + 1) / 2;
        }
      P.n_valid = 128; P.out_planes = 2;
      for (int p = 0; p < 2; ++p) P.out_p[p] = v.dZ1[p];
      P.mask = v.H1[n][0];
      P.colsum = h->g(std::string(nets[n]) + "/cnn1/b"); P.colsum_mask = 31;
      g.host[g.n++] = P;
    }
    if (int rc = push_group(h, v.bwd_groups, g, "conv2_dgrad")) return rc;
  }
  {
    CgGroup g;
    for (int n = 0; n < 2; ++n) {
      const int mA = add_maps(v, v.H1[n], NB, 4, {64, 14, 15, (uint64_t)B}, {64, 15 * 64, 225 * 64}, {64, 12, 12, 4}, {1, 2, 2, 1});
      const int mB = add_maps(v, v.dZ2[n], NB, 2, {64, (uint64_t)B * 36}, {128}, {64, 144});
      if (mA < 0 || mB < 0) return b2g_fail(B2G_ECUDA, "engine v2: cuTensorMapEncodeTiled failed (conv2 wgrad)");
      CgProblem P = mnmajor(NB, 144, 2, 1, (B + 3) / 4);
      P.nloads = 3;
      for (int a = 0; a < 2; ++a) { P.ld[a] = mk_load(mA, 4, a * P.a_lbo); P.ld[a].c0[1] = 2 * a; P.ld[a].d_tm[2] = 1; P.ld[a].d_c2[3] = 4; }
      P.ld[2] = mk_load(mB, 2, P.b_off); P.ld[2].d_c2[1] = 144;
      P.tiles_m = 4; P.tiles_n = 1;
      P.splits = std::max(1, std::min(P.chunks, std::max(8, (P.chunks + 7) / 8)));
      P.lim_rows = 512; P.o_tm = 128 * 64; P.o0 = 64; P.n_valid = 64;
      P.out_f = h->g(std::string(nets[n]) + "/cnn2/w"); P.atomic = 1;
      g.host[g.n++] = P;
    }
    {
      const int mA = add_maps(v, v.A1[0], NB, 2, {(uint64_t)K1, (uint64_t)B * 225}, {(uint64_t)K1 * 2}, {64, 64});
      const int mB = add_maps(v, v.dZ1, NB, 2, {64, (uint64_t)B * 225}, {128}, {64, 64});
      if (mA < 0 || mB < 0) return b2g_fail(B2G_ECUDA, "engine v2: cuTensorMapEncodeTiled failed (conv1 wgrad)");
      CgProblem P = mnmajor(NB, 64, 2, 1, (B * 225 + 63) / 64);
      P.nloads = 3;
      for (int a = 0; a < 2; ++a) { P.ld[a] = mk_load(mA, 2, a * P.a_lbo); P.ld[a].c0[0] = 64 * a; P.ld[a].d_tm[0] = 128; P.ld[a].d_c2[1] = 64; }
      P.ld[2] = mk_load(mB, 2, P.b_off); P.ld[2].d_c2[1] = 64;
      P.tiles_m = (K1 + 127) / 128; P.tiles_n = 1;
      P.splits = std::max(1, std::min(P.chunks, std::max(84 / P.tiles_m, (P.chunks + 15) / 16)));
      P.lim_rows = K1; P.o_tm = 128 * 32; P.o0 = 32; P.n_valid = 64;
      P.out_f = h->g("model/pi/cnn1/w"); P.f_grp = (long long)(h->g("model/values_fn/cnn1/w") - h->g("model/pi/cnn1/w")); P.atomic = 1;
      g.host[g.n++] = P;
    }
    if (int rc = push_group(h, v.bwd_groups, g, "conv_wgrad")) return rc;
  }
  int n_ctr = 0;
  {
    std::vector<const CgGroup*> parts;
    for (auto& g : v.fwd) parts.push_back(&g);
    std::vector<Wire> w;
    for (int n = 0; n < 3; ++n) {
      w.push_back({1, n, 0, n < 2 ? 0 : 1, 3 * 225, 128, 0});
      w.push_back({2, n, 1, n, 8 * 36, 108, 0});
      w.push_back({3, n, 2, n, 128 * 16, 128, 0});
      w.push_back({4, n, 3, n, 128, 128, 0});
    }
    if (int rc = fuse_groups(h, parts, w, "fwd_fused", v.fwd_fused, n_ctr)) return rc;
  }
  {
    std::vector<const CgGroup*> parts;
    for (auto& g : v.bwd_groups) parts.push_back(&g);
    std::vector<Wire> w;
    for (int n = 0; n < 2; ++n) {
      w.push_back({1, 2 * n, 0, n, 128, 128, 0});
      w.push_back({1, 2 * n + 1, 0, n, 64, 128, 1});
      w.push_back({2, 2 * n, 1, 2 * n, 3, 128, 0});
      w.push_back({2, 2 * n + 1, 1, 2 * n, 4, 128, 1});
      w.push_back({3, n, 2, 2 * n, 72, 108, 0});
      w.push_back({4, n, 2, 2 * n, 144, 108, 1});
    }
    w.push_back({4, 2, 3, 0, 64, 450, 1});
    w.push_back({4, 2, 3, 1, 64, 450, 1});
    if (int rc = fuse_groups(h, parts, w, "bwd_fused", v.bwd_fused, n_ctr)) return rc;
    std::vector<const CgGroup*> pa(parts.begin(), parts.begin() + 2), pb(parts.begin() + 2, parts.end());
    std::vector<Wire> wa, wb;
    for (int n = 0; n < 2; ++n) {
      wa.push_back({1, 2 * n, 0, n, 128, 128, 0});
      wa.push_back({1, 2 * n + 1, 0, n, 64, 128, 1});
      wb.push_back({1, n, 0, 2 * n, 72, 108, 0});
      wb.push_back({2, n, 0, 2 * n, 144, 108, 1});
    }
    wb.push_back({2, 2, 1, 0, 64, 450, 1});
    wb.push_back({2, 2, 1, 1, 64, 450, 1});
    if (int rc = fuse_groups(h, pa, wa, "bwd_fused_fc", v.bwd_fused, n_ctr)) return rc;
    if (int rc = fuse_groups(h, pb, wb, "bwd_fused_conv", v.bwd_fused, n_ctr)) return rc;
  }
  if (int rc = dev_alloc(h->allocs, h->stream, &v.dep_ctr, (size_t)n_ctr)) return rc;
  v.n_dep_ctr = n_ctr;
  bind_counters(v.fwd_fused, v.dep_ctr);
  bind_counters(v.bwd_fused, v.dep_ctr);
  if (int rc = dev_alloc(h->allocs, h->stream, &v.d_maps, v.maps.size())) return rc;
  CK(cudaMemcpyAsync(v.d_maps, v.maps.data(), v.maps.size() * sizeof(CUtensorMap), cudaMemcpyHostToDevice, h->stream));
  CK(cudaStreamSynchronize(h->stream));
  return 0;
}

int v2_planes(b2g_sac* h, cudaStream_t s) {
  V2State& v = h->v2;
  planes2_kernel<<<v.plane_ctas, 256, 0, s>>>((const Plane2Job*)v.plane_jobs, v.plane_cta_job);
  return 0;
}

int v2_gather(b2g_sac* h, const GatherArgs& ga, cudaStream_t s) {
  V2State& v = h->v2;
  Gather2Args a{};
  a.g = ga;
  for (int w = 0; w < 2; ++w)
    for (int p = 0; p < 3; ++p) a.a1[w][p] = v.A1[w][p];
  for (int n = 0; n < 3; ++n) for (int p = 0; p < 3; ++p) a.fp[n][p] = v.F[n][p];
  a.KF = v.KF; a.Ci = h->Cimg; a.OH = h->H1; a.OW = h->W1;
  const size_t smem = (size_t)3 * h->Hi * (h->Wi * h->Cimg + 8) * sizeof(uint16_t);
  static size_t attr = 0;
  if (smem > attr) {
    CK(cudaFuncSetAttribute(gather2_kernel, cudaFuncAttributeMaxDynamicSharedMemorySize, (int)smem));
    attr = smem;
  }
  gather2_kernel<<<dim3(ga.B, ga.next_obs || ga.next_frame ? 2 : 1), 512, smem, s>>>(a);
  return 0;
}

extern long long* g_cg_trace;
static long long* s_trace_buf = nullptr;

int v2_launch(b2g_sac* h, const CgGroup& g, cudaStream_t s) {
  const char* tn = getenv("B2G_CG_TRACE");
  cudaStreamCaptureStatus cs0 = cudaStreamCaptureStatusNone;
  if (tn) cudaStreamIsCapturing(s, &cs0);
  if (tn && cs0 == cudaStreamCaptureStatusNone && std::string(tn) == g.name) {
    if (!s_trace_buf) cudaMalloc(&s_trace_buf, 640 * sizeof(long long));
    cudaMemsetAsync(s_trace_buf, 0, 640 * sizeof(long long), s);
    g_cg_trace = s_trace_buf;
    const char* tc = getenv("B2G_CG_TRACE_CTA");
    cudaError_t e = cg_launch(g, h->v2.d_maps, h->num_sms - h->v2.sm_reserve, s, false, h->v2.dbg | ((tc ? atoi(tc) : 0) << 8));
    g_cg_trace = nullptr;
    if (e != cudaSuccess) return b2g_fail(B2G_ECUDA, cudaGetErrorString(e));
    static int shots = 0;
    if (shots++ == 3) {
      long long t[640];
      cudaStreamSynchronize(s);
      cudaMemcpy(t, s_trace_buf, sizeof(t), cudaMemcpyDeviceToHost);
      const long long t0 = t[0];
      fprintf(stderr, "cg trace %s (cycles; per chunk: prod wait_start wait_done issued | mma wait_start full_seen committed)\n", g.name);
      for (int i = 0; i < 64 && t[i * 8 + 2]; ++i)
        fprintf(stderr, "  chunk %2d (p %lld tm %lld): %7lld %7lld %7lld | %7lld %7lld %7lld\n", i, t[i * 8 + 6] / 100000, t[i * 8 + 6] % 100000 / 10, t[i * 8] - t0,
                t[i * 8 + 1] - t0, t[i * 8 + 2] - t0, t[i * 8 + 3] - t0, t[i * 8 + 4] - t0, t[i * 8 + 5] - t0);
      for (int i = 0; i < 16 && t[512 + i * 4 + 1]; ++i)
        fprintf(stderr, "  tile %d (p %lld tm %lld) mma: start %7lld sums out %7lld (%s)\n", i, t[512 + i * 4 + 3] / 100000, t[512 + i * 4 + 3] % 100000 / 10,
                t[512 + i * 4] - t0, t[512 + i * 4 + 1] - t0, t[512 + i * 4 + 2] ? "handed off" : "in place");
      for (int i = 0; i < 16 && t[576 + i * 4 + 2]; ++i)
        fprintf(stderr, "  handoff %d (p %lld tm %lld) epilogue warpgroup: buffer wait %7lld start %7lld end %7lld\n", i, t[576 + i * 4 + 3] / 100000,
                t[576 + i * 4 + 3] % 100000 / 10, t[576 + i * 4] - t0, t[576 + i * 4 + 1] - t0, t[576 + i * 4 + 2] - t0);
    }
    return 0;
  }
  CK(cg_launch(g, h->v2.d_maps, h->num_sms - h->v2.sm_reserve, s, pdl_enabled(), h->v2.dbg));
  return 0;
}

}
```

### deep-rl-grasping_b200/csrc/sac.cu

```cuda
#include <cuda_runtime.h>
#include <math.h>
#include <stdio.h>
#include <string.h>

#include <algorithm>
#include <chrono>
#include <map>
#include <tuple>
#include <string>
#include <vector>

#include "../../include/b200grasp.h"
#include "common.cuh"
#include "sac_internal.cuh"

using namespace b2g;

namespace b2g {
bool pdl_enabled() {
  static int v = -1;
  if (v < 0) { const char* e = getenv("B2G_PDL"); v = (e && e[0] == '0') ? 0 : 1; }
  return v != 0;
}
}
// ... 724 lines not shown
    h->v2.sm_reserve = 0;
  } else {
    int last_fc1 = -1;
    for (size_t i = 0; i < h->bwd_groups.size(); ++i)
      if (h->bwd_groups[i].name.find("fc1") != std::string::npos || h->bwd_groups[i].name.find("heads") != std::string::npos) last_fc1 = (int)i;
    for (size_t i = 0; i < h->bwd_groups.size(); ++i) {
      const bool leaf = fork && h->bwd_groups[i].name == "heads_wgrad";
      if (fork && h->use_planes && i + 1 == h->bwd_groups.size()) {
        CK(cudaEventRecord(h->ev_aux[4], s)); CK(cudaStreamWaitEvent(ax, h->ev_aux[4], 0));
        colsum_launch(h->d_colsum, h->n_colsum, h->colsum_ctas, ax); ++n;
      }
      if (leaf) {
        CK(cudaEventRecord(h->ev_aux[2], s));
        CK(cudaStreamWaitEvent(ax, h->ev_aux[2], 0));
      }
      if (int rc = run_group(h->bwd_groups[i], leaf ? ax : s)) return rc;
      if ((int)i == last_fc1) {
        if (fork) { CK(cudaEventRecord(h->ev_aux[3], s)); CK(cudaStreamWaitEvent(ax, h->ev_aux[3], 0)); }
        if (h->use_planes && h->n_colsum_early) {
          colsum_launch(h->d_colsum_early, h->n_colsum_early, h->colsum_early_ctas, ax); ++n; mark("bias_grads_fc1");
        }
      }
    }
    if (h->use_planes && !fork) { colsum_launch(h->d_colsum, h->n_colsum, h->colsum_ctas, s); ++n; mark("bias_grads"); }
  }
  if (fork) { CK(cudaEventRecord(h->ev_aux[5], ax)); CK(cudaStreamWaitEvent(s, h->ev_aux[5], 0)); }
  if (h->cfg.nranks > 1 && !(h->dp_p2p && apply)) {
    if (overlap) {
      if (int rc = nccl_ck(g_nccl.GroupStart())) return rc;
      if (int rc = nccl_ck(g_nccl.AllReduce(h->G, h->G, (size_t)pi_fc1, 7, 0, h->nccl_comm, s))) return rc;
      if (int rc = nccl_ck(g_nccl.AllReduce(h->G + h->n_pi, h->G + h->n_pi, (size_t)(v_fc1 - h->n_pi), 7, 0, h->nccl_comm, s))) return rc;
      if (int rc = nccl_ck(g_nccl.GroupEnd())) return rc;
      ++n;
      CK(cudaStreamWaitEvent(s, h->ev_join, 0));
    } else {
      CK(cudaMemcpyAsync(h->G + h->n_train, h->metrics, MET_GN_PI * sizeof(float), cudaMemcpyDeviceToDevice, s)); ++n_copy;
      if (int rc = nccl_ck(g_nccl.AllReduce(h->G, h->G, (size_t)(h->n_train + MET_COUNT),  7,  0, h->nccl_comm, s))) return rc;
      ++n;
    }
    CK(cudaMemcpyAsync(h->metrics, h->G + h->n_train, MET_GN_PI * sizeof(float), cudaMemcpyDeviceToDevice, s)); ++n_copy;
    mark("allreduce");
  }
  OptimArgs oa = make_optim();
  oa.bump_counter = (fork && sampled) ? h->counters + 4 : nullptr;
  if (dp_early_opt) {
    oa.r_lo[0] = 0; oa.r_hi[0] = (int)pi_fc1;
    oa.r_lo[1] = (int)h->n_pi; oa.r_hi[1] = (int)v_fc1;
  }
  if (h->dp_p2p && apply) {
    DpArgs da{};
    da.o = oa; da.rank = h->cfg.rank; da.nranks = h->cfg.nranks;
    for (int q = 0; q < h->cfg.nranks; ++q) { da.R_peer[q] = h->dp_G[q]; da.P_peer[q] = h->dp_P[q]; da.x_peer[q] = h->dp_X[q]; }
    da.counters = h->counters; da.sync = h->dp_sync;
    for (int k = 0; k < 2; ++k) { da.skip_lo4[k] = h->dp_skip[k][0]; da.skip_hi4[k] = h->dp_skip[k][1]; }
    dp_optim_launch(da, h->num_sms, s); ++n;
    mark("adam_polyak_dp");
  } else {
    optim_launch(oa, s); ++n; mark("adam_polyak");
  }
  if (h->use_planes && apply && !h->v2.on) {
    if (!fork) { planes_launch(h->d_jobs, h->n_jobs, h->job_tiles, s); ++n; mark("weight_planes"); }
  }
  CK(cudaGetLastError());
  if (n_launch) *n_launch = n;
  return 0;
}

void refresh_planes(b2g_sac* h, bool for_step = false) {
  if (for_step && (h->fork_leaves || h->v2.on)) {
    h->planes_dirty = true;
    return;
  }
  if (h->use_planes && h->planes_dirty) {
    planes_launch(h->d_jobs, h->n_jobs, h->job_tiles, h->stream);
    h->planes_dirty = false;
  }
}

void fill_metrics(const b2g_sac* h, const float* m, const long long* cnt, b2g_sac_metrics* out) {
  const float inv = 1.0f / (float)h->cfg.nranks;
  out->policy_loss = m[MET_POLICY_LOSS] * inv; out->qf1_loss = m[MET_QF1_LOSS] * inv; out->qf2_loss = m[MET_QF2_LOSS] * inv;
  out->value_loss = m[MET_VALUE_LOSS] * inv; out->ent_coef_loss = m[MET_ENT_COEF_LOSS] * inv; out->entropy = m[MET_ENTROPY] * inv;
  out->mean_q1 = m[MET_MEAN_Q1] * inv; out->mean_q2 = m[MET_MEAN_Q2] * inv; out->mean_v = m[MET_MEAN_V] * inv;
  out->mean_logp = m[MET_MEAN_LOGP] * inv;
  out->grad_norm_pi = sqrtf(m[MET_GN_PI]); out->grad_norm_values = sqrtf(m[MET_GN_VALUES]);
  out->grad_ent = m[MET_COUNT + 1] * inv;
  out->ent_coef = expf(m[MET_COUNT]);
  out->n_updates = cnt[3];
}

int copy_metrics_async(b2g_sac* h, float* met, long long* cnt) {
  CK(cudaMemcpyAsync(met, h->metrics, MET_COUNT * sizeof(float), cudaMemcpyDeviceToHost, h->stream));
  CK(cudaMemcpyAsync(met + MET_COUNT, h->p("model/log_ent_coef"), sizeof(float), cudaMemcpyDeviceToHost, h->stream));
  CK(cudaMemcpyAsync(met + MET_COUNT + 1, h->g("model/log_ent_coef"), sizeof(float), cudaMemcpyDeviceToHost, h->stream));
  CK(cudaMemcpyAsync(cnt, h->counters, 8 * sizeof(long long), cudaMemcpyDeviceToHost, h->stream));
  return 0;
}

int fetch_metrics(b2g_sac* h, b2g_sac_metrics* out) {
  if (int rc = copy_metrics_async(h, h->h_met, h->h_cnt)) return rc;
  CK(cudaStreamSynchronize(h->stream));
  if (out) fill_metrics(h, h->h_met, h->h_cnt, out);
  return 0;
}

int find_tensor(const b2g_sac* h, const char* name) {
  if (!name) return -1;
  std::string n(name);
  if (n.size() > 2 && n.compare(n.size() - 2, 2, ":0") == 0) n.resize(n.size() - 2);
  auto it = h->tindex.find(n);
  return it == h->tindex.end() ? -1 : it->second;
}

int full_index(const b2g_sac* h, int e) {
  if (!h->cnn) return e;
  const int Ci = h->Cimg, npx = h->Hi * h->Wi * Ci;
  if (e < npx) return (e / Ci) * (Ci + 1) + e % Ci;
  return e == npx ? Ci : -1;
}

int load_rows(b2g_sac* h, const float* src, float* dst, long long first, long long wrap, long long n) {
  const size_t E = h->E;
  if (!h->cnn) {
    CK(cudaMemcpyAsync(dst + first * E, src, n * E * sizeof(float), cudaMemcpyDefault, h->stream));
    return 0;
  }
  for (long long i = 0; i < n; i += h->stage_rows) {
    const int m = (int)std::min<long long>(h->stage_rows, n - i);
    CK(cudaMemcpyAsync(h->obs_stage, src + i * E, m * E * sizeof(float), cudaMemcpyDefault, h->stream));
    compact_rows(h->obs_stage, dst, first + i, wrap, m, h->Hi * h->Wi, h->Cimg + 1, h->stream);
  }
  return 0;
}

}

extern "C" {

int b2g_sac_dp_export(b2g_sac* h, void* out192) {
  if (!h || !out192) return b2g_fail(B2G_EINVAL, "b2g_sac_dp_export: null argument");
  cudaSetDevice(h->cfg.device);
  if (!h->dp_x) {
    if (int rc = dev_alloc(h->allocs, h->stream, &h->dp_x, 256)) return rc;
    if (int rc = dev_alloc(h->allocs, h->stream, &h->dp_recv, h->n_train + 64 * DP_MAX_RANKS)) return rc;
    if (int rc = dev_alloc(h->allocs, h->stream, &h->dp_sync, 64)) return rc;
    CK(cudaStreamSynchronize(h->stream));
  }
  cudaIpcMemHandle_t hd[3];
  CK(cudaIpcGetMemHandle(&hd[0], h->P));
  CK(cudaIpcGetMemHandle(&hd[1], h->dp_recv));
  CK(cudaIpcGetMemHandle(&hd[2], h->dp_x));
  static_assert(sizeof(hd) == B2G_DP_EXPORT_BYTES, "export blob size");
  memcpy(out192, hd, sizeof(hd));
  return 0;
}

int b2g_debug_dp_stamps(b2g_sac* h, long long* out5) {
  if (!h || !h->dp_sync) return b2g_fail(B2G_EINVAL, "b2g_debug_dp_stamps: not connected");
  CK(cudaStreamSynchronize(h->stream));
  CK(cudaMemcpy(out5, h->dp_sync + 8, 5 * sizeof(long long), cudaMemcpyDeviceToHost));
  return 0;
}

int b2g_sac_dp_connect(b2g_sac* h, const void* all_exports, int nranks) {
  if (!h || !all_exports) return b2g_fail(B2G_EINVAL, "b2g_sac_dp_connect: null argument");
  if (nranks != h->cfg.nranks || nranks < 2 || nranks > DP_MAX_RANKS) return b2g_fail(B2G_EINVAL, "b2g_sac_dp_connect: nranks must equal the learner's (2..8)");
  if (!h->dp_x) return b2g_fail(B2G_EINVAL, "b2g_sac_dp_connect: call b2g_sac_dp_export first");
  if (h->dp_p2p) return b2g_fail(B2G_ESTATE, "b2g_sac_dp_connect: already connected");
  if (((h->n_pi | h->n_values | h->n_ent | h->n_target) & 3) != 0) return b2g_fail(B2G_EINVAL, "b2g_sac_dp_connect: arena segments are not float4 aligned");
  cudaSetDevice(h->cfg.device);
  CK(cudaStreamSynchronize(h->stream));
  for (int q = 0; q < nranks; ++q) {
    if (q == h->cfg.rank) { h->dp_P[q] = h->P; h->dp_G[q] = h->dp_recv; h->dp_X[q] = h->dp_x; continue; }
    cudaIpcMemHandle_t hd[3];
    memcpy(hd, (const char*)all_exports + (size_t)q * B2G_DP_EXPORT_BYTES, sizeof(hd));
    void* p[3] = {nullptr, nullptr, nullptr};
    for (int k = 0; k < 3; ++k) {
      CK(cudaIpcOpenMemHandle(&p[k], hd[k], cudaIpcMemLazyEnablePeerAccess));
      h->dp_opened.push_back(p[k]);
    }
    h->dp_P[q] = (float*)p[0]; h->dp_G[q] = (float*)p[1]; h->dp_X[q] = (int*)p[2];
  }
  h->dp_skip[0][0] = h->dp_skip[0][1] = h->dp_skip[1][0] = h->dp_skip[1][1] = 0;
  if (h->v2.on) {
    const int n_train4 = (int)((h->n_pi + h->n_values + h->n_ent) >> 2), per4 = (n_train4 + nranks - 1) / nranks;
    const char* names[2] = {"model/pi/cnn_fc1/w", "model/values_fn/cnn_fc1/w"};
    for (int k = 0; k < 2; ++k) {
      const float* gp = h->g(names[k]);
      const auto& t = h->tensors[h->tindex.at(names[k])];
      bool found = false;
      auto patch = [&](std::vector<CgGroup>& groups) {
        for (CgGroup& g : groups)
          for (int i = 0; i < g.n; ++i) {
            CgProblem& P = g.host[i];
            if (P.epi != CG_EPI_WGRAD || P.atomic || P.out_f != gp) continue;
            for (int q = 0; q < nranks; ++q) P.dp_recv[q] = h->dp_G[q];
            P.dp_gbase = h->G; P.dp_rank = h->cfg.rank; P.dp_n = nranks; P.dp_per4 = per4;
            found = true;
          }
      };
      patch(h->v2.bwd_fused);
      if (found && (t.off & 3) == 0) { h->dp_skip[k][0] = (int)(t.off >> 2); h->dp_skip[k][1] = (int)((t.off + 1024 * 512) >> 2); }
    }
  }
  h->dp_p2p = true;
  if (h->graph_exec) { cudaGraphExecDestroy(h->graph_exec); h->graph_exec = nullptr; }
  for (auto& g : h->pipe_graph) if (g) { cudaGraphExecDestroy(g); g = nullptr; }
  return 0;
}

int b2g_sac_destroy(b2g_sac* h) {
  if (!h) return 0;
  cudaSetDevice(h->cfg.device);
  if (h->stream) cudaStreamSynchronize(h->stream);
  if (h->graph_exec) cudaGraphExecDestroy(h->graph_exec);
  for (auto& g : h->pipe_graph) if (g) cudaGraphExecDestroy(g);
  for (void* q : h->dp_opened) cudaIpcCloseMemHandle(q);
  nccl_comm_destroy(h->nccl_comm2);
  nccl_comm_destroy(h->nccl_comm);
  if (h->side) cudaStreamDestroy(h->side);
  if (h->aux) { cudaStreamSynchronize(h->aux); cudaStreamDestroy(h->aux); }
  for (auto& e : h->ev_aux) if (e) cudaEventDestroy(e);
  if (h->ev_fork) cudaEventDestroy(h->ev_fork);
  if (h->ev_join) cudaEventDestroy(h->ev_join);
  for (void* q : h->allocs) cudaFree(q);
  for (int q = 0; q < 2; ++q) { if (h->hc_obs[q]) cudaFreeHost(h->hc_obs[q]); if (h->hc_next[q]) cudaFreeHost(h->hc_next[q]); }
  if (h->h_met) cudaFreeHost(h->h_met);
  if (h->h_cnt) cudaFreeHost(h->h_cnt);
  if (h->h_plan) cudaFreeHost(h->h_plan);
  if (h->h_rc) cudaFreeHost(h->h_rc);
  for (int k = 0; k < 2; ++k) { if (h->hp_stats[k]) cudaFreeHost(h->hp_stats[k]); if (h->ev_stats[k]) cudaEventDestroy(h->ev_stats[k]); }
  for (int j = 0; j < 2; ++j) {
    if (h->ev_h2d[j]) cudaEventDestroy(h->ev_h2d[j]);
    if (h->ev_consumed[j]) cudaEventDestroy(h->ev_consumed[j]);
    if (h->ev_met[j]) cudaEventDestroy(h->ev_met[j]);
    if (h->pm_met[j]) cudaFreeHost(h->pm_met[j]);
    if (h->pm_cnt[j]) cudaFreeHost(h->pm_cnt[j]);
  }
  if (h->cstream) cudaStreamDestroy(h->cstream);
  if (h->ev0) cudaEventDestroy(h->ev0);
  if (h->ev1) cudaEventDestroy(h->ev1);
  if (h->stream) cudaStreamDestroy(h->stream);
  delete h;
  return 0;
}

int b2g_sac_create(const b2g_sac_cfg* cfg, b2g_sac** out) { return b2g_sac_create2(cfg, nullptr, out); }

int b2g_sac_create2(const b2g_sac_cfg* cfg, const b2g_replay_cfg* replay, b2g_sac** out) {
  if (!cfg || !out) return b2g_fail(B2G_EINVAL, "cfg/out is NULL");
  *out = nullptr;
  if (replay && replay->frame_capacity < cfg->buffer_capacity + 1)
    return b2g_fail(B2G_EINVAL, "frame_capacity must be at least buffer_capacity + 1");
  if (replay && replay->u8_plane_mask && cfg->obs_h <= 0) return b2g_fail(B2G_EINVAL, "the MLP policy has no 8-bit image planes");
  if (replay && replay->u8_plane_mask &&
      (cfg->obs_c < 2 || cfg->obs_c - 1 > 8 || (replay->u8_plane_mask >> (cfg->obs_c - 1)) != 0))
    return b2g_fail(B2G_EINVAL, "u8_plane_mask may only name image planes, at most 8 (the actuator plane is the last channel)");
  if (cfg->hidden != 64 && cfg->hidden != 128 && cfg->hidden != 192 && cfg->hidden != 256)
    return b2g_fail(B2G_EINVAL, "hidden must be 64, 128, 192 or 256 (SAC.layers [H, H])");
  if (cfg->n_act < 1 || cfg->n_act > 8) return b2g_fail(B2G_EINVAL, "n_act must be in [1,8]");
  if (cfg->batch < 1 || cfg->buffer_capacity < 1) return b2g_fail(B2G_EINVAL, "batch and buffer_capacity must be positive");
  if (cfg->nranks < 1 || cfg->rank < 0 || cfg->rank >= cfg->nranks) return b2g_fail(B2G_EINVAL, "bad rank/nranks");
  if (cfg->precision < B2G_PREC_FP32_SIMT || cfg->precision > B2G_PREC_BF16)
    return b2g_fail(B2G_EINVAL, "unknown precision mode");
  int num_sms = 0;
  if (int rc = check_device(cfg->device, &num_sms)) return rc;

  b2g_sac* h = new b2g_sac();
  h->cfg = *cfg;
  h->num_sms = num_sms;
  h->cfg.nccl_id = nullptr; h->cfg.nccl_lib = nullptr;
  h->cnn = cfg->obs_h > 0;
  h->B = cfg->batch; h->A = cfg->n_act; h->H = cfg->hidden;
  if (h->cnn) {
    if (cfg->obs_c < 2) { delete h; return b2g_fail(B2G_EINVAL, "CNN policy needs obs_c >= 2 (image planes + feature plane)"); }
    h->Cimg = cfg->obs_c - 1; h->Hi = cfg->obs_h; h->Wi = cfg->obs_w;
    h->H1 = (h->Hi - 8) / 4 + 1; h->W1 = (h->Wi - 8) / 4 + 1;
    h->H2 = (h->H1 - 4) / 2 + 1; h->W2 = (h->W1 - 4) / 2 + 1;
    h->H3 = h->H2 - 2; h->W3 = h->W2 - 2;
    if (h->H3 * h->W3 * 64 != 1024 || (h->Wi * h->Cimg) % 4 != 0) {
      delete h;
      return b2g_fail(B2G_EINVAL, "observation size must give a 4x4x64 conv3 output (64x64 input; cnn_fc1/w is (1024,512))");
    }
    h->E = h->Hi * h->Wi * cfg->obs_c;
    h->Ec = h->Hi * h->Wi * h->Cimg + 4;
    h->feat_dim = 513;
  } else {
    if (cfg->obs_dim < 1) { delete h; return b2g_fail(B2G_EINVAL, "obs_dim must be positive for the MLP policy"); }
    h->E = h->Ec = cfg->obs_dim;
    h->feat_dim = cfg->obs_dim;
  }
  h->FS = (h->feat_dim + h->A + 7) / 8 * 8;
  auto bail = [&](int rc) { std::string keep = g_b2g_err; b2g_sac_destroy(h); g_b2g_err = keep; return rc; };
  if (cudaStreamCreateWithFlags(&h->stream, cudaStreamNonBlocking) != cudaSuccess) return bail(b2g_fail(B2G_ECUDA, "cudaStreamCreate failed"));
  cudaEventCreate(&h->ev0); cudaEventCreate(&h->ev1);
  build_params(h);
  int rc = 0;
  const int B = h->B;
#define DA(ptr, count) if ((rc = dev_alloc(h->allocs, h->stream, &(ptr), (size_t)(count)))) return bail(rc)
  DA(h->P, h->n_all); DA(h->Mo, h->n_train); DA(h->Vo, h->n_train); DA(h->G, h->n_train + MET_COUNT);
  DA(h->metrics, MET_COUNT); DA(h->counters, 8); DA(h->step_consts, 4); DA(h->d_lr, 1);
  const int64_t cap = cfg->buffer_capacity;
  {
    h->v2.on = h->cnn && cfg->precision == B2G_PREC_BF16X3 && h->Hi == 64 && h->Wi == 64;
    if (const char* dbg = getenv("B2G_CG_DEBUG")) h->v2.dbg = atoi(dbg);
  }
  {
    const int npx = h->cnn ? h->Hi * h->Wi * h->Cimg : 0, HW = h->Hi * h->Wi;
    h->row_fmt.n32 = h->Cimg; h->row_fmt.tail = 4 * npx;
    h->u8_mask = replay ? replay->u8_plane_mask : 0;
    h->fmt = h->row_fmt;
    h->frame_bytes = (int64_t)h->Ec * 4;
    if (h->u8_mask) {
      FrameFmt& f = h->fmt;
      f.n8 = f.n32 = 0;
      for (int c = 0; c < h->Cimg; ++c) f.ch[c] = (h->u8_mask >> c & 1) ? (signed char)f.n8++ : (signed char)(-1 - f.n32++);
      f.f32_off = HW * f.n8;
      f.tail = f.f32_off + 4 * HW * f.n32;
      if (f.f32_off % 16 != 0) return bail(b2g_fail(B2G_EINVAL, "8-bit planes need H * W * (8-bit planes) to be a multiple of 16"));
      h->frame_bytes = (f.tail + 16 + 15) / 16 * 16;
    }
    h->frame_cap = replay ? replay->frame_capacity : 2 * cap;
    if (h->frame_cap > INT32_MAX) return bail(b2g_fail(B2G_EINVAL, "frame_capacity must fit in int32 (frame indices)"));
    h->dedup = h->frame_cap < 2 * cap;
  }
  if ((rc = dev_alloc(h->allocs, h->stream, &h->frames, (size_t)(h->frame_cap * h->frame_bytes)))) return bail(rc);
  DA(h->r_ofr, cap); DA(h->r_nfr, cap); DA(h->r_act, cap * h->A); DA(h->r_rew, cap); DA(h->r_done, cap);
  h->stage_rows = std::max(B, 256);
  if (h->cnn) DA(h->obs_stage, (size_t)h->stage_rows * h->E);
  DA(h->c_obs, (size_t)h->stage_rows * h->Ec); DA(h->c_next, (size_t)h->stage_rows * h->Ec); DA(h->d_plan, 4 * h->stage_rows);
  if (cudaMallocHost((void**)&h->h_plan, 4 * h->stage_rows * sizeof(int)) != cudaSuccess ||
      cudaMallocHost((void**)&h->h_rc, 2 * sizeof(long long)) != cudaSuccess)
    return bail(b2g_fail(B2G_ECUDA, "replay staging"));
  DA(h->d_mean, h->Ec); DA(h->d_istd, h->Ec); DA(h->d_normc, 8);
  for (int k = 0; k < 2; ++k) {
    if (cudaMallocHost((void**)&h->hp_stats[k], (size_t)(2 * h->Ec + 8) * sizeof(double)) != cudaSuccess ||
        cudaEventCreateWithFlags(&h->ev_stats[k], cudaEventDisableTiming) != cudaSuccess)
      return bail(b2g_fail(B2G_ECUDA, "norm-stat staging"));
  }
  DA(h->s_obs, (size_t)B * h->Ec); DA(h->s_next, (size_t)B * h->Ec); DA(h->s_act, B * h->A); DA(h->s_rew, B); DA(h->s_done, B);
  if (h->cnn) {
    DA(h->x_obs, (size_t)B * h->Hi * h->Wi * h->Cimg); DA(h->x_next, (size_t)B * h->Hi * h->Wi * h->Cimg);
    for (int n = 0; n < 3; ++n) {
      DA(h->h1[n], (size_t)B * h->H1 * h->W1 * 32); DA(h->h2[n], (size_t)B * h->H2 * h->W2 * 64); DA(h->h3[n], (size_t)B * 1024);
    }
    for (int n = 0; n < 2 && !h->v2.on; ++n) {
      DA(h->dZ4[n], (size_t)B * 512); DA(h->dZ3p[n], (size_t)B * (h->H3 + 4) * (h->W3 + 4) * 64);
      DA(h->dZ2p[n], (size_t)B * (h->H2 + 3) * (h->W2 + 3) * 64); DA(h->dZ1[n], (size_t)B * h->H1 * h->W1 * 32);
    }
  }
  h->use_planes = h->cnn && cfg->precision != B2G_PREC_FP32_SIMT;
  if (h->v2.on && (rc = v2_alloc(h))) return bail(rc);
  if (h->use_planes) {
    const size_t nx = (size_t)B * h->Hi * h->Wi * h->Cimg;
    for (int k = 0; k < 2; ++k) { DA(h->xp[0][k], nx); DA(h->xp[1][k], nx); }
    for (int n = 0; n < 3; ++n)
      for (int k = 0; k < 2; ++k) {
        if (h->v2.on) {
          h->h1p[n][k] = h->v2.H1[n][k]; h->h2p[n][k] = h->v2.H2[n][k]; h->h3p[n][k] = h->v2.H3[n][k];
          continue;
        }
        DA(h->h1p[n][k], (size_t)B * h->H1 * h->W1 * 32); DA(h->h2p[n][k], (size_t)B * h->H2 * h->W2 * 64); DA(h->h3p[n][k], (size_t)B * 1024);
      }
    for (int n = 0; n < 2 && !h->v2.on; ++n)
      for (int k = 0; k < 2; ++k) {
        DA(h->dZ4p[n][k], (size_t)B * 512); DA(h->dZ3pp[n][k], (size_t)B * (h->H3 + 4) * (h->W3 + 4) * 64);
        DA(h->dZ2pp[n][k], (size_t)B * (h->H2 + 3) * (h->W2 + 3) * 64);
        DA(h->dZ1p[n][k], (size_t)B * h->H1 * h->W1 * 32);
      }
    const size_t wsz[4] = {(size_t)64 * h->Cimg * 32, 512 * 64, 576 * 64, 1024 * 512};
    for (int n = 0; n < 3; ++n)
      for (int l = 0; l < 4; ++l)
        for (int k = 0; k < 4; ++k) {
          if (n == 2 && k < 2) continue;
          DA(h->wp[n][l][k], wsz[l]);
        }
  }
  for (int n = 0; n < 3; ++n) DA(h->F[n], (size_t)B * h->FS);
  DA(h->z0[0], 5 * B * h->H);
  for (int q = 1; q < 5; ++q) h->z0[q] = h->z0[0] + (size_t)q * B * h->H;
  for (int q = 0; q < 4; ++q) { DA(h->a0[q], B * h->H); DA(h->dz1[q], B * h->H); }
  DA(h->dz0_pi, B * h->H); DA(h->dz0_v3, B * 3 * h->H);
  DA(h->per_sample, 7 * B); DA(h->pi_out, B * h->A); DA(h->eps, B * h->A + 4); DA(h->rew_n, B); DA(h->done_n, B);
  DA(h->indices, B + 4);
#undef DA
  if (cudaMallocHost((void**)&h->h_met, (MET_COUNT + 2) * sizeof(float)) != cudaSuccess ||
      cudaMallocHost((void**)&h->h_cnt, 8 * sizeof(long long)) != cudaSuccess)
    return bail(b2g_fail(B2G_ECUDA, "cudaMallocHost failed"));
  for (int j = 0; j < 2; ++j) {
    if ((rc = dev_alloc(h->allocs, h->stream, &h->ps_obs[j], (size_t)B * h->Ec)) || (rc = dev_alloc(h->allocs, h->stream, &h->ps_next[j], (size_t)B * h->Ec))) return bail(rc);
    if (cudaEventCreateWithFlags(&h->ev_h2d[j], cudaEventDisableTiming) != cudaSuccess ||
        cudaEventCreateWithFlags(&h->ev_consumed[j], cudaEventDisableTiming) != cudaSuccess ||
        cudaEventCreateWithFlags(&h->ev_met[j], cudaEventDisableTiming) != cudaSuccess ||
        cudaMallocHost((void**)&h->pm_met[j], (MET_COUNT + 2) * sizeof(float)) != cudaSuccess ||
        cudaMallocHost((void**)&h->pm_cnt[j], 8 * sizeof(long long)) != cudaSuccess)
      return bail(b2g_fail(B2G_ECUDA, "pipelined-path resources"));
  }
  if (cudaStreamCreateWithFlags(&h->cstream, cudaStreamNonBlocking) != cudaSuccess) return bail(b2g_fail(B2G_ECUDA, "copy stream"));
  {
    const char* fk = getenv("B2G_FORK");
    if (!(fk && atoi(fk) == 0)) {
      if (cudaStreamCreateWithFlags(&h->aux, cudaStreamNonBlocking) != cudaSuccess) return bail(b2g_fail(B2G_ECUDA, "aux stream"));
      for (auto& e : h->ev_aux)
        if (cudaEventCreateWithFlags(&e, cudaEventDisableTiming) != cudaSuccess) return bail(b2g_fail(B2G_ECUDA, "aux events"));
      h->fork_leaves = true;
    }
  }
  {
    std::vector<double> ones(h->Ec, 1.0);
    if (cudaMemcpyAsync(h->d_istd, ones.data(), h->Ec * sizeof(double), cudaMemcpyHostToDevice, h->stream) != cudaSuccess ||
        cudaStreamSynchronize(h->stream) != cudaSuccess)
      return bail(b2g_fail(B2G_ECUDA, "init copy failed"));
  }
  if ((rc = build_groups(h))) return bail(rc);
  if (h->v2.on && (rc = v2_create(h))) return bail(rc);
  if (cfg->nranks > 1) {
    if (!cfg->nccl_id) return bail(b2g_fail(B2G_EINVAL, "nranks > 1 needs nccl_id"));
    if ((rc = nccl_comm_init(&h->nccl_comm, cfg->nranks, cfg->nccl_id, cfg->rank, cfg->nccl_lib))) return bail(rc);
    {
      const char* ov = getenv("B2G_AR_OVERLAP");
      const bool want_ov = h->v2.on && !(ov && ov[0] == '0');
      if (want_ov && g_nccl.CommSplit && g_nccl.GroupStart && g_nccl.GroupEnd) {
        if (g_nccl.CommSplit(h->nccl_comm, 0, cfg->rank, &h->nccl_comm2, nullptr) == 0 && h->nccl_comm2 &&
            cudaStreamCreateWithFlags(&h->side, cudaStreamNonBlocking) == cudaSuccess &&
            cudaEventCreateWithFlags(&h->ev_fork, cudaEventDisableTiming) == cudaSuccess &&
            cudaEventCreateWithFlags(&h->ev_join, cudaEventDisableTiming) == cudaSuccess) {
          h->overlap_ar = true;
          if (const char* e = getenv("B2G_AR_SMS")) h->ar_sms = atoi(e);
          g_nccl.AllReduce(h->G, h->G, 1024, 7, 0, h->nccl_comm2, h->side);
          cudaStreamSynchronize(h->side);
        }
      }
    }
    const int nrc = g_nccl.AllReduce(h->G, h->G, (size_t)(h->n_train + MET_COUNT), 7, 0, h->nccl_comm, h->stream);
    if (nrc != 0 || cudaStreamSynchronize(h->stream) != cudaSuccess) return bail(b2g_fail(B2G_ENCCL, "NCCL warm-up all-reduce failed"));
  }
  const char* ng = getenv("B2G_NO_GRAPH");
  h->use_graph = !(ng && ng[0] == '1');
  if (cudaStreamSynchronize(h->stream) != cudaSuccess) return bail(b2g_fail(B2G_ECUDA, "create: sync failed"));
  *out = h;
  return 0;
}

int b2g_sync(b2g_sac* h) {
  if (!h) return b2g_fail(B2G_EINVAL, "NULL handle");
  CK(cudaSetDevice(h->cfg.device));
  CK(cudaStreamSynchronize(h->stream));
  return 0;
}

int b2g_param_count(const b2g_sac* h) { return h ? (int)h->tensors.size() : 0; }

int b2g_param_info(const b2g_sac* h, int idx, const char** name, int64_t* numel, int32_t* ndim, int64_t shape[4]) {
  if (!h || idx < 0 || idx >= (int)h->tensors.size()) return b2g_fail(B2G_EINVAL, "bad tensor index");
  const Tensor& t = h->tensors[idx];
  if (name) *name = t.name.c_str();
  if (numel) *numel = t.numel;
  if (ndim) *ndim = t.ndim;
  if (shape) for (int i = 0; i < 4; ++i) shape[i] = t.shape[i];
  return 0;
}

static int copy_tensor(b2g_sac* h, const char* name, float* arena, float* host, size_t numel, bool to_host, bool trainable_only) {
  if (!h || !host) return b2g_fail(B2G_EINVAL, "NULL argument");
  const int i = find_tensor(h, name);
  if (i < 0) return b2g_fail(B2G_EINVAL, std::string("unknown variable: ") + (name ? name : "(null)"));
  const Tensor& t = h->tensors[i];
  if ((int64_t)numel != t.numel) return b2g_fail(B2G_EINVAL, std::string("size mismatch for ") + t.name);
  if (trainable_only && t.group == 3) return b2g_fail(B2G_EINVAL, std::string("not a trainable variable: ") + t.name);
  CK(cudaSetDevice(h->cfg.device));
  CK(cudaStreamSynchronize(h->stream));
  if (to_host) CK(cudaMemcpy(host, arena + t.off, numel * sizeof(float), cudaMemcpyDeviceToHost));
  else CK(cudaMemcpy(arena + t.off, host, numel * sizeof(float), cudaMemcpyHostToDevice));
  return 0;
}

int b2g_get_param(b2g_sac* h, const char* name, float* dst, size_t numel) { return copy_tensor(h, name, h ? h->P : nullptr, dst, numel, true, false); }
int b2g_set_param(b2g_sac* h, const char* name, const float* src, size_t numel) {
  int rc = copy_tensor(h, name, h ? h->P : nullptr, const_cast<float*>(src), numel, false, false);
  if (rc == 0) h->planes_dirty = true;
  return rc;
}
int b2g_get_grad(b2g_sac* h, const char* name, float* dst, size_t numel) {
  int rc = copy_tensor(h, name, h ? h->G : nullptr, dst, numel, true, true);
  if (rc == 0 && h->cfg.nranks > 1) for (size_t i = 0; i < numel; ++i) dst[i] /= (float)h->cfg.nranks;
  return rc;
}
int b2g_get_adam(b2g_sac* h, const char* name, float* m, float* v, size_t numel) {
  if (int rc = copy_tensor(h, name, h ? h->Mo : nullptr, m, numel, true, true)) return rc;
  return copy_tensor(h, name, h->Vo, v, numel, true, true);
}
int b2g_reset_optimizer(b2g_sac* h) {
  if (!h) return b2g_fail(B2G_EINVAL, "NULL handle");
  CK(cudaSetDevice(h->cfg.device));
  CK(cudaMemsetAsync(h->Mo, 0, h->n_train * sizeof(float), h->stream));
  CK(cudaMemsetAsync(h->Vo, 0, h->n_train * sizeof(float), h->stream));
  CK(cudaMemsetAsync(h->counters, 0, 4 * sizeof(long long), h->stream));
  CK(cudaStreamSynchronize(h->stream));
  return 0;
}

int b2g_replay_add(b2g_sac* h, const float* obs, const float* act, const float* rew, const float* next_obs, const float* done,
                   int64_t n) {
  if (!h || !obs || !act || !rew || !next_obs || !done || n < 0) return b2g_fail(B2G_EINVAL, "NULL argument");
  if (h->dedup && 2 * n > h->frame_cap) return b2g_fail(B2G_EINVAL, "replay_add: 2 n rows exceed frame_capacity");
  CK(cudaSetDevice(h->cfg.device));
  const int64_t cap = h->cfg.buffer_capacity, FC = h->frame_cap;
  const int64_t R = std::min<int64_t>({(int64_t)h->stage_rows, cap, FC / 2});
  const size_t E = h->E, A = h->A;
  FrameIo io{};
  io.c_obs = h->c_obs; io.c_next = h->c_next; io.frames = h->frames; io.frame_bytes = h->frame_bytes;
  io.fmt = h->fmt; io.npx = h->cnn ? h->Hi * h->Wi * h->Cimg : 0; io.Ci = h->cnn ? h->Cimg : 1; io.Ec = h->Ec;
  int* flags = h->h_plan + 3 * R;
  auto stage_check = [&](int64_t c0, int m, bool check) -> int {
    if (c0 > 0) CK(cudaStreamSynchronize(h->stream));
    if (int rc = load_rows(h, obs + c0 * E, h->c_obs, 0, R, m)) return rc;
    if (int rc = load_rows(h, next_obs + c0 * E, h->c_next, 0, R, m)) return rc;
    if (!check) return 0;
    for (int i = 0; i < m; ++i) {
      const int64_t p = c0 + i < (int64_t)h->prev_next.size() ? h->prev_next[c0 + i] : -1;
      h->h_plan[i] = h->dedup && p >= 0 && p > h->next_fid - FC ? (int)(p % FC) : -1;
    }
    CK(cudaMemcpyAsync(h->d_plan, h->h_plan, m * sizeof(int), cudaMemcpyHostToDevice, h->stream));
    frame_check_launch(io, h->d_plan, h->d_plan + 3 * R, m, h->stream);
    CK(cudaMemcpyAsync(flags, h->d_plan + 3 * R, m * sizeof(int), cudaMemcpyDeviceToHost, h->stream));
    CK(cudaStreamSynchronize(h->stream));
    for (int i = 0; i < m; ++i)
      if (flags[i] & 2) return b2g_fail(B2G_EINVAL, "replay_add: a value of an 8-bit plane is not an integer in [0, 255]");
    return 0;
  };
  if (h->u8_mask && n > R)
    for (int64_t c0 = 0; c0 < n; c0 += R)
      if (int rc = stage_check(c0, (int)std::min<int64_t>(R, n - c0), true)) return rc;
  auto alloc_frame = [&]() -> int64_t {
    const int64_t f = h->next_fid++, over = f - FC;
    while (h->head_seq > h->tail_seq) {
      while (h->lw.front().first < h->tail_seq) h->lw.pop_front();
      if (h->lw.front().second > over) break;
      ++h->tail_seq; ++h->evicted;
    }
    return f;
  };
  std::vector<int64_t> next_ids((size_t)n);
  for (int64_t c0 = 0; c0 < n; c0 += R) {
    const int m = (int)std::min<int64_t>(R, n - c0);
    if (int rc = stage_check(c0, m, h->dedup || (h->u8_mask && n <= R))) return rc;
    const int64_t first = h->head_seq, fid0 = h->next_fid;
    for (int i = 0; i < m; ++i) {
      if (h->head_seq - h->tail_seq == cap) ++h->tail_seq;
      const int64_t p = c0 + i < (int64_t)h->prev_next.size() ? h->prev_next[c0 + i] : -1;
      const bool share = h->dedup && (flags[i] & 1) && p >= h->next_fid + 1 - FC;
      const int64_t of = share ? p : alloc_frame();
      const int64_t nf = alloc_frame();
      while (!h->lw.empty() && h->lw.back().second >= of) h->lw.pop_back();
      h->lw.emplace_back(h->head_seq++, of);
      h->h_plan[i] = (int)(of % FC); h->h_plan[m + i] = share ? 0 : 1; h->h_plan[2 * m + i] = (int)(nf % FC);
      next_ids[c0 + i] = nf;
    }
    if (h->dedup) CK(cudaMemcpyAsync(h->d_plan, h->h_plan, 3 * m * sizeof(int), cudaMemcpyHostToDevice, h->stream));
    frame_commit_launch(io, h->dedup ? h->d_plan : nullptr, fid0, FC, m, h->r_ofr, h->r_nfr, first, cap, h->stream);
    for (int64_t k = 0; k < m;) {
      const int64_t pos = (first + k) % cap, len = std::min<int64_t>(m - k, cap - pos);
      CK(cudaMemcpyAsync(h->r_act + pos * A, act + (c0 + k) * A, len * A * sizeof(float), cudaMemcpyDefault, h->stream));
      CK(cudaMemcpyAsync(h->r_rew + pos, rew + c0 + k, len * sizeof(float), cudaMemcpyDefault, h->stream));
      CK(cudaMemcpyAsync(h->r_done + pos, done + c0 + k, len * sizeof(float), cudaMemcpyDefault, h->stream));
      k += len;
    }
  }
  h->prev_next.swap(next_ids);
  h->r_size = h->head_seq - h->tail_seq;
  h->h_rc[0] = h->r_size;
  h->h_rc[1] = h->r_size == cap ? 0 : h->tail_seq % cap;
  CK(cudaMemcpyAsync(h->counters + 5, h->h_rc, 2 * sizeof(long long), cudaMemcpyHostToDevice, h->stream));
  CK(cudaStreamSynchronize(h->stream));
  return 0;
}

int64_t b2g_replay_size(const b2g_sac* h) { return h ? h->r_size : 0; }

int b2g_replay_info(const b2g_sac* h, int64_t* capacity, int64_t* size, int64_t* frame_capacity, int64_t* live_frames,
                    int64_t* bytes, int64_t* evicted_early) {
  if (!h) return b2g_fail(B2G_EINVAL, "NULL handle");
  const int64_t cap = h->cfg.buffer_capacity;
  int64_t live = 0;
  if (h->r_size > 0) {
    int64_t lo = h->next_fid;
    for (const auto& q : h->lw) if (q.first >= h->tail_seq) { lo = q.second; break; }
    live = h->next_fid - lo;
  }
  if (capacity) *capacity = cap;
  if (size) *size = h->r_size;
  if (frame_capacity) *frame_capacity = h->frame_cap;
  if (live_frames) *live_frames = live;
  if (bytes) *bytes = h->frame_cap * h->frame_bytes + cap * (int64_t)(2 * sizeof(int) + (h->A + 2) * sizeof(float));
  if (evicted_early) *evicted_early = h->evicted;
  return 0;
}

int b2g_replay_get(b2g_sac* h, int64_t slot, float* obs, float* act, float* rew, float* next_obs, float* done) {
  if (!h) return b2g_fail(B2G_EINVAL, "NULL handle");
  const int64_t cap = h->cfg.buffer_capacity;
  if (slot < 0 || slot >= cap || ((slot - h->tail_seq % cap) % cap + cap) % cap >= h->r_size)
    return b2g_fail(B2G_EINVAL, "replay slot is not live");
  CK(cudaSetDevice(h->cfg.device));
  CK(cudaStreamSynchronize(h->stream));
  const size_t A = h->A;
  std::vector<unsigned char> fr(h->frame_bytes);
// ... 306 lines not shown
```

### deep-rl-grasping_b200/csrc/sac_internal.cuh

```cuda
#pragma once
#include <cuda_runtime.h>

#include <deque>
#include <map>
#include <string>
#include <tuple>
#include <vector>

#include "../../include/b200grasp.h"
#include "cg.cuh"
#include "common.cuh"
#include "host.cuh"

namespace b2g {
struct Tensor {
  std::string name;
  int ndim;
  int64_t shape[4];
  int64_t numel;
  int64_t off;
  int group;
};


struct V2State {
  bool on = false;
  int KF = 576;
  uint16_t* A1[2][3]{};
  uint16_t* H1[3][3]{};
  uint16_t* H2[3][3]{};
  uint16_t* H3[3][3]{};
  uint16_t* F[3][3]{};
  uint16_t* dz0pi[2]{};
  uint16_t* dz0v[2]{};
  uint16_t* dZ4[2][2]{};
  uint16_t* dZ3[2][2]{};
  uint16_t* dZ2[2][2]{};
  uint16_t* dZ1[2]{};
  uint16_t* W1T[2][3]{};
  uint16_t* W2T[3][3]{};
  uint16_t* W3T[3][3]{};
  uint16_t* WfT[3][3]{};
  uint16_t* K0T[3][3]{};
  uint16_t* W2n[2][2]{};
  uint16_t* W3n[2][2]{};
  uint16_t* Wfn[2][2]{};
  uint16_t* K0n[2][2]{};
  float* z0v = nullptr;
  void* plane_jobs = nullptr; int n_plane_jobs = 0, plane_ctas = 0;
  const int* plane_cta_job = nullptr;
  int sm_reserve = 0;
  std::vector<CUtensorMap> maps;
  std::vector<char> map_whole;
  std::vector<int> map_box_bytes;
  CUtensorMap* d_maps = nullptr;
  std::vector<CgGroup> fwd, bwd_groups;
  std::vector<CgGroup> fwd_fused, bwd_fused;
  int split_fc1 = 3;
  int split_fc1_dgrad = 1;
  int* dep_ctr = nullptr; int n_dep_ctr = 0;
  std::vector<int*> tabs;
  int dbg = 0;
};

}

struct b2g_sac;
namespace b2g {
int v2_alloc(b2g_sac* h);
int v2_create(b2g_sac* h);
int v2_planes(b2g_sac* h, cudaStream_t s);
int v2_gather(b2g_sac* h, const GatherArgs& ga, cudaStream_t s);
int v2_launch(b2g_sac* h, const CgGroup& g, cudaStream_t s);
}

using namespace b2g;

struct b2g_sac {
  b2g_sac_cfg cfg{};
  bool cnn = false;
  int num_sms = 132;
  int B = 0, A = 0, H = 0, E = 0, Cimg = 0, feat_dim = 0, FS = 0;
  int Hi = 0, Wi = 0, H1 = 0, W1 = 0, H2 = 0, W2 = 0, H3 = 0, W3 = 0;
  std::vector<Tensor> tensors;
  std::map<std::string, int> tindex;
  int64_t n_pi = 0, n_values = 0, n_ent = 0, n_target = 0, n_train = 0, n_all = 0;
  float *P = nullptr, *Mo = nullptr, *Vo = nullptr, *G = nullptr;
  float* metrics = nullptr;
  cudaStream_t stream = nullptr;
  std::vector<void*> allocs;
  int Ec = 0;
  unsigned char* frames = nullptr;
  int64_t frame_cap = 0, frame_bytes = 0;
  FrameFmt fmt{}, row_fmt{};
  uint32_t u8_mask = 0;
  bool dedup = false;
  int *r_ofr = nullptr, *r_nfr = nullptr;
  float *r_act = nullptr, *r_rew = nullptr, *r_done = nullptr;
  int64_t r_size = 0, head_seq = 0, tail_seq = 0, next_fid = 0, evicted = 0;
  std::deque<std::pair<int64_t, int64_t>> lw;
  std::vector<int64_t> prev_next;
  float *c_obs = nullptr, *c_next = nullptr;
  int *d_plan = nullptr, *h_plan = nullptr;
  long long* h_rc = nullptr;
  float* obs_stage = nullptr;
  int stage_rows = 0;
  double *d_mean = nullptr, *d_istd = nullptr, *d_normc = nullptr;
  double ret_istd = 1.0, clip_obs = 10.0, clip_rew = 10.0;
  int norm_obs = 0, norm_rew = 0;
  float *x_obs = nullptr, *x_next = nullptr;
  float *h1[3]{}, *h2[3]{}, *h3[3]{}, *F[3]{};
  float *dZ4[2]{}, *dZ3p[2]{}, *dZ2p[2]{}, *dZ1[2]{};
  float *z0[5]{}, *a0[4]{}, *dz1[4]{}, *dz0_pi = nullptr, *dz0_v3 = nullptr;
  bool use_planes = false;
  uint16_t *xp[2][2]{}, *h1p[3][2]{}, *h2p[3][2]{}, *h3p[3][2]{};
  uint16_t *dZ4p[2][2]{}, *dZ3pp[2][2]{}, *dZ2pp[2][2]{}, *dZ1p[2][2]{};
  ColsumJob* d_colsum = nullptr;
  int n_colsum = 0, colsum_ctas = 0;
  uint16_t* wp[3][4][4]{};
  PlaneJob* d_jobs = nullptr;
  int n_jobs = 0, job_tiles = 0;
  bool planes_dirty = true;
  std::map<const int*, std::vector<int>> host_tabs;
  float *per_sample = nullptr, *pi_out = nullptr, *eps = nullptr, *rew_n = nullptr, *done_n = nullptr;
  int* indices = nullptr;
  float *s_obs = nullptr, *s_next = nullptr, *s_act = nullptr, *s_rew = nullptr, *s_done = nullptr;
  float *ps_obs[2]{}, *ps_next[2]{};
  float *hc_obs[2]{}, *hc_next[2]{};
  cudaGraphExec_t pipe_graph[2]{};
  int host_threads = 16;
  cudaStream_t cstream = nullptr;
  cudaEvent_t ev_h2d[2]{}, ev_consumed[2]{}, ev_met[2]{};
  float* pm_met[2]{};
  long long* pm_cnt[2]{};
  long long pipe_k = 0;
  bool pipe_pending = false;
  cudaEvent_t record_after_gather = nullptr;
  long long* counters = nullptr;
  double* step_consts = nullptr;
  float* d_lr = nullptr;
  float cur_lr = -1.f;
  std::vector<GemmGroup> fwd_groups, bwd_groups, act_groups;
  cudaGraphExec_t graph_exec = nullptr;
  bool use_graph = true;
  void* nccl_comm = nullptr;
  void* nccl_comm2 = nullptr;
  bool pipe_serial = false; int pipe_tune = 0; double pipe_t0 = 0, pipe_period[2] = {0, 0};
  bool dp_p2p = false;
  int* dp_x = nullptr;
  int* dp_sync = nullptr;
  float* dp_recv = nullptr;
  float* dp_P[8]{}; float* dp_G[8]{}; int* dp_X[8]{};
  std::vector<void*> dp_opened;
  int dp_skip[2][2]{};
  cudaStream_t side = nullptr;
  cudaStream_t aux = nullptr;
  cudaEvent_t ev_aux[7]{};
  bool fork_leaves = false;
  std::map<std::tuple<const void*, const void*, const void*, int>, int> col_ids;
  cudaEvent_t ev_fork = nullptr, ev_join = nullptr;
  bool overlap_ar = false;
  int ar_sms = 8;
  ColsumJob* d_colsum_early = nullptr;
  int n_colsum_early = 0, colsum_early_ctas = 0;
  cudaEvent_t ev0 = nullptr, ev1 = nullptr;
  float last_ms = 0.f;
  int launches = 0;
  std::vector<std::string> prof_names;
  float* h_met = nullptr;
  long long* h_cnt = nullptr;

  b2g::V2State v2;
  double* hp_stats[2]{};
  cudaEvent_t ev_stats[2]{};
  int stats_k = 0;

  float* p(const std::string& n) { return P + tensors[tindex.at(n)].off; }
  float* g(const std::string& n) { return G + tensors[tindex.at(n)].off; }
};
```

Measured before the change: 2243.

## Replace materialized conv1 im2col with space-to-depth layout read directly by TMA

The gather kernel no longer builds an explicit im2col matrix through shared memory. It writes the observation in a space-to-depth (4x4 block) bf16x3 plane layout instead. Conv1 forward and its weight gradient now load patches straight from that layout with 3D/4D TMA boxes, using precomputed wgmma descriptor bits, optional 64B swizzle, and new epilogue row-group and sub-tile offsets. Conv1 weights are permuted to match. This removes the 225x-overlapping im2col write and read traffic, at the cost of more complex addressing, wasted padded rows (16x16 tiles for a 15x15 output), and new correctness risk in the index math.

```diff
diff --git a/deep-rl-grasping_b200/csrc/cg.cu b/deep-rl-grasping_b200/csrc/cg.cu
--- a/deep-rl-grasping_b200/csrc/cg.cu
+++ b/deep-rl-grasping_b200/csrc/cg.cu
@@ -49,8 +49,7 @@
       : "=r"(pred));
   return pred != 0;
 }
-__device__ __forceinline__ uint64_t desc_k(uint32_t saddr) { return wg_desc(saddr, 16, 1024); }
-__device__ __forceinline__ uint64_t desc_mn(uint32_t saddr, uint32_t lbo) { return wg_desc(saddr, lbo, 1024); }
+__device__ __forceinline__ uint64_t desc_at(uint64_t bits, uint32_t saddr) { return bits | (uint64_t)((saddr & 0x3FFFFu) >> 4); }
 
 __device__ __forceinline__ void tma_load(uint32_t dst, const CUtensorMap* map, uint32_t bar, int rank, const int (&c)[5]) {
   switch (rank) {
@@ -115,7 +114,7 @@
 
 template <int NT, int NPROD, int TRANS, int KS, int NACC>
 __device__ __forceinline__ void mma_chunk(float (&acc)[NACC], uint32_t sbase, uint32_t a_off, uint32_t b_off, uint32_t a_ks, uint32_t b_ks,
-                                          uint32_t a_lbo, uint32_t b_lbo, uint32_t a_ps, uint32_t b_ps, uint32_t m_off) {
+                                          uint32_t a_ks2, uint64_t a_desc, uint64_t b_desc, uint32_t a_ps, uint32_t b_ps, uint32_t m_off) {
   constexpr int NPL = NPROD >= 6 ? 3 : (NPROD >= 3 ? 2 : 1), G = NT / 2;
   static_assert(NACC == G * NPL, "one accumulator group of NT columns per product order");
 #pragma unroll
@@ -123,10 +122,10 @@
     uint64_t da[NPL], db[NPL];
 #pragma unroll
     for (int pl = 0; pl < NPL; ++pl) {
-      const uint32_t pa = sbase + (uint32_t)pl * a_ps + a_off + (uint32_t)k * a_ks + m_off;
+      const uint32_t pa = sbase + (uint32_t)pl * a_ps + a_off + (uint32_t)(k & 1) * a_ks + (uint32_t)(k >> 1) * a_ks2 + m_off;
       const uint32_t pb = sbase + (uint32_t)pl * b_ps + b_off + (uint32_t)k * b_ks;
-      da[pl] = TRANS ? desc_mn(pa, a_lbo) : desc_k(pa);
-      db[pl] = TRANS ? desc_mn(pb, b_lbo) : desc_k(pb);
+      da[pl] = desc_at(a_desc, pa);
+      db[pl] = desc_at(b_desc, pb);
     }
     Wgmma<NT, TRANS>::mma(acc, da[0], db[0]);
     if constexpr (NPL >= 2) Wgmma<NT, TRANS>::mma(acc + G, da[0], db[1]);
@@ -172,8 +171,9 @@
 #pragma unroll
   for (int j = 0; j < NACC; ++j) acc[j] = 0.f;
   const uint32_t a_ps = (uint32_t)P.a_pstride, b_ps = (uint32_t)P.b_pstride, a_off = P.a_off, b_off = P.b_off, a_ks = P.a_kstep, b_ks = P.b_kstep;
-  const uint32_t a_lbo = P.a_lbo, b_lbo = P.b_lbo;
-  const uint32_t m_off = TRANS ? (uint32_t)wg * a_lbo : (uint32_t)wg * 8192u;
+  const uint32_t a_ks2 = P.a_kstep2;
+  const uint64_t a_desc = P.a_desc, b_desc = P.b_desc;
+  const uint32_t m_off = (uint32_t)wg * (uint32_t)P.a_moff;
   uint32_t prev = 0;
   if (nomma) {
     for (int c = ti.c_begin; c < ti.c_end; ++c, ++gc) {
@@ -190,7 +190,7 @@
       mbar_wait(smem_u32(&bar_full[s]), (ph >> s) & 1u);
       stamp_if(tr + 4, stamp);
       wg_arrive();
-      mma_chunk<NT, NPROD, TRANS, KS>(acc, ring + s * (uint32_t)slot_bytes, a_off, b_off, a_ks, b_ks, a_lbo, b_lbo, a_ps, b_ps, m_off);
+      mma_chunk<NT, NPROD, TRANS, KS>(acc, ring + s * (uint32_t)slot_bytes, a_off, b_off, a_ks, b_ks, a_ks2, a_desc, b_desc, a_ps, b_ps, m_off);
       wg_commit();
       wg_wait<1>();
       mbar_arrive_if(smem_u32(&bar_empty[prev]), lane == 0 && c > ti.c_begin);
@@ -263,12 +263,15 @@
 struct RowOff {
   long long roff = 0, rmoff = 0;
   int ri0 = 0, ri1 = 0;
+  bool ok = true;
   __device__ __forceinline__ void set(const CgProblem& Q, int r) {
     const int d0 = Q.d0, d1 = Q.d1;
     const int i0 = r % d0, i12 = r / d0, i1 = i12 % d1, i2 = i12 / d1;
     roff = Q.o_base + (long long)i0 * Q.o0 + (long long)i1 * Q.o1 + (long long)i2 * Q.o2;
+    if (Q.rgrp_rows > 0) roff += Q.rgrp_off[min(r / Q.rgrp_rows, 7)];
     rmoff = Q.m_base + (long long)i0 * Q.m0 + (long long)i1 * Q.m1 + (long long)i2 * Q.m2;
     ri0 = i0; ri1 = i1;
+    ok = Q.lim_i0 <= 0 || i0 < Q.lim_i0;
   }
 };
 
@@ -414,7 +417,7 @@
       const Tile ti = w.tile(tile);
       if (ti.c_end <= ti.c_begin) continue;
       const CgProblem& P = probs[ti.p];
-      const bool valid0 = r < rows_tile && ti.tm * rows_tile + r < lim_rows;
+      const bool valid0 = r < rows_tile && ti.tm * rows_tile + r < lim_rows && ro.ok;
       const long long off0 = ro.roff + (long long)ti.tm * o_tm;
       const int n0 = ti.tn * umma_n;
       const bool tre = trace && blockIdx.x == trace_cta && warp == 0 && lane == 0 && it < 16;
@@ -507,8 +510,14 @@
       const Tile ti = w.tile(tile);
       if (ti.c_end <= ti.c_begin || !handoff) continue;
       const CgProblem& P = probs[ti.p];
-      const bool valid0 = r < rows_tile && ti.tm * rows_tile + r < lim_rows;
-      const long long off0 = ro.roff + (long long)ti.tm * o_tm, moff0 = ro.rmoff + (long long)ti.tm * m_tm;
+      bool valid0 = r < rows_tile && ti.tm * rows_tile + r < lim_rows && ro.ok;
+      long long off0 = ro.roff + (long long)ti.tm * o_tm;
+      const long long moff0 = ro.rmoff + (long long)ti.tm * m_tm;
+      if (P.tm_sub > 1) {
+        const int tq = ti.tm / P.tm_sub, tr = ti.tm - tq * P.tm_sub;
+        off0 = ro.roff + (long long)tq * o_tm + (long long)tr * P.o_sub;
+        valid0 = valid0 && tr * P.d1 + ro.ri1 < P.lim_i1;
+      }
       const int n0 = ti.tn * umma_n, ngroups = umma_n >> 5;
       auto group_at = [&](int g, bool& valid, long long& off, long long& moff) {
         const int ng = n0 + 32 * g;
@@ -682,7 +691,8 @@
 int cg_smem_limit() { return 226 * 1024 - STG_BYTES; }
 
 int cg_encode_map(CUtensorMap* out, const void* base, int rank, const uint64_t* dims, const uint64_t* strides_bytes, const uint32_t* box,
-                  const uint32_t* elem_strides) {
+                  const uint32_t* elem_strides, int swizzle) {
+  if (swizzle != 128 && swizzle != 64) return -1;
   if (!g_encode) {
     cudaDriverEntryPointQueryResult q;
     void* fn = nullptr;
@@ -694,8 +704,14 @@
   for (int i = 0; i < rank; ++i) { gd[i] = dims[i]; bx[i] = box[i]; es[i] = elem_strides ? elem_strides[i] : 1; }
   for (int i = 0; i + 1 < rank; ++i) gs[i] = strides_bytes[i];
   const CUresult r = g_encode(out, CU_TENSOR_MAP_DATA_TYPE_BFLOAT16, (cuuint32_t)rank, const_cast<void*>(base), gd, gs, bx, es, CU_TENSOR_MAP_INTERLEAVE_NONE,
-                              CU_TENSOR_MAP_SWIZZLE_128B, CU_TENSOR_MAP_L2_PROMOTION_L2_256B, CU_TENSOR_MAP_FLOAT_OOB_FILL_NONE);
+                              swizzle == 128 ? CU_TENSOR_MAP_SWIZZLE_128B : CU_TENSOR_MAP_SWIZZLE_64B, CU_TENSOR_MAP_L2_PROMOTION_L2_256B,
+                              CU_TENSOR_MAP_FLOAT_OOB_FILL_NONE);
   return r == CUDA_SUCCESS ? 0 : (int)r;
+}
+
+unsigned long long cg_desc_bits(int swizzle, bool mn_major, int lbo) {
+  const unsigned long long l = mn_major ? (unsigned)lbo : 16u, sbo = 8u * (unsigned)swizzle;
+  return ((l >> 4) & 0x3FFF) << 16 | ((sbo >> 4) & 0x3FFF) << 32 | (unsigned long long)(swizzle == 128 ? 1 : 2) << 62;
 }
 
 int cg_finalize(CgGroup& g, int smem_budget) {
diff --git a/deep-rl-grasping_b200/csrc/cg.cuh b/deep-rl-grasping_b200/csrc/cg.cuh
--- a/deep-rl-grasping_b200/csrc/cg.cuh
+++ b/deep-rl-grasping_b200/csrc/cg.cuh
@@ -41,9 +41,12 @@
   CgLoad ld[CG_MAX_LOADS];
   const int* tm_tab;
   int mn_major;
+  unsigned long long a_desc, b_desc;
+  int a_moff;
   int ksteps;
   int a_off, b_off;
   int a_kstep, b_kstep;
+  int a_kstep2;
   int a_lbo, b_lbo;
   int umma_n;
   int nprod;
@@ -52,6 +55,12 @@
   int lim_rows;
   int d0, d1;
   long long o_tm; int o0, o1, o2; long long o_base;
+  int rgrp_rows;
+  int rgrp_off[8];
+  int lim_i0;
+  int tm_sub;
+  long long o_sub;
+  int lim_i1;
   long long m_tm; int m0, m1, m2; long long m_base;
   int n_valid;
   int grp_stride;
@@ -90,7 +99,8 @@
 };
 
 int cg_encode_map(CUtensorMap* out, const void* base, int rank, const uint64_t* dims, const uint64_t* strides_bytes, const uint32_t* box,
-                  const uint32_t* elem_strides);
+                  const uint32_t* elem_strides, int swizzle = 128);
+unsigned long long cg_desc_bits(int swizzle, bool mn_major, int lbo);
 int cg_finalize(CgGroup& g, int smem_budget);
 cudaError_t cg_launch(const CgGroup& g, const CUtensorMap* dev_maps, int num_sms, cudaStream_t s, bool pdl, int debug_flags);
 int cg_smem_limit();
diff --git a/deep-rl-grasping_b200/csrc/engine_v2.cu b/deep-rl-grasping_b200/csrc/engine_v2.cu
--- a/deep-rl-grasping_b200/csrc/engine_v2.cu
+++ b/deep-rl-grasping_b200/csrc/engine_v2.cu
@@ -12,9 +12,9 @@
 
 struct Gather2Args {
   GatherArgs g;
-  uint16_t* a1[2][3];
+  uint16_t* s1[2][3];
   uint16_t* fp[3][3];
-  int KF, Ci, OH, OW;
+  int KF;
 };
 
 __device__ __forceinline__ void split3(float y, uint16_t& p0, uint16_t& p1, uint16_t& p2) {
@@ -25,11 +25,67 @@
   p0 = __bfloat16_as_ushort(h0); p1 = __bfloat16_as_ushort(h1); p2 = __bfloat16_as_ushort(__float2bfloat16_rn(r2));
 }
 
+template <int Ci>
+__device__ __forceinline__ void s2d_half_block(const Gather2Args& a, const unsigned char* __restrict__ src, int it, int which, size_t b) {
+  constexpr int CP = s2d_channels(Ci);
+  const GatherArgs& g = a.g;
+  const int npx = g.H * g.W * Ci;
+  const int h = it & 1, X = (it >> 1) & 15, Y = it >> 5;
+  const double clip_obs = g.normc[1];
+  const bool norm_obs = g.normc[3] != 0.0;
+  const float scale = g.scale;
+#pragma unroll
+  for (int rr = 0; rr < 2; ++rr) {
+    const int e0 = ((4 * Y + 2 * h + rr) * g.W + 4 * X) * Ci;
+    float y[4 * Ci];
+#pragma unroll
+    for (int q = 0; q < Ci; ++q) {
+      const int e = e0 + 4 * q;
+      const float4 v = frame_load4(src, g.fmt, npx, Ci, e);
+      float t[4] = {v.x, v.y, v.z, v.w};
+      if (norm_obs) {
+        const double2 m0 = *reinterpret_cast<const double2*>(g.mean + e), m1 = *reinterpret_cast<const double2*>(g.mean + e + 2);
+        const double2 i0 = *reinterpret_cast<const double2*>(g.var + e), i1 = *reinterpret_cast<const double2*>(g.var + e + 2);
+        t[0] = (float)fmin(fmax(((double)t[0] - m0.x) * i0.x, -clip_obs), clip_obs);
+        t[1] = (float)fmin(fmax(((double)t[1] - m0.y) * i0.y, -clip_obs), clip_obs);
+        t[2] = (float)fmin(fmax(((double)t[2] - m1.x) * i1.x, -clip_obs), clip_obs);
+        t[3] = (float)fmin(fmax(((double)t[3] - m1.y) * i1.y, -clip_obs), clip_obs);
+      }
+#pragma unroll
+      for (int j = 0; j < 4; ++j) y[4 * q + j] = t[j];
+    }
+    uint32_t p[3][2 * CP];
+#pragma unroll
+    for (int k = 0; k < 4 * CP; k += 2) {
+      uint16_t q[3][2];
+#pragma unroll
+      for (int u = 0; u < 2; ++u) {
+        const int c = (k + u) / CP, ci = (k + u) % CP;
+        if (ci < Ci) split3(y[c * Ci + ci] / scale, q[0][u], q[1][u], q[2][u]);
+        else q[0][u] = q[1][u] = q[2][u] = 0;
+      }
+#pragma unroll
+      for (int pl = 0; pl < 3; ++pl) p[pl][k / 2] = (uint32_t)q[pl][0] | ((uint32_t)q[pl][1] << 16);
+    }
+    const size_t o = b * 4096 * CP + (size_t)((Y * 16 + X) * 16 + 4 * (2 * h + rr)) * CP;
+#pragma unroll
+    for (int pl = 0; pl < 3; ++pl) {
+      if constexpr (CP == 1) {
+        *reinterpret_cast<uint2*>(a.s1[which][pl] + o) = make_uint2(p[pl][0], p[pl][1]);
+      } else {
+        uint4* d = reinterpret_cast<uint4*>(a.s1[which][pl] + o);
+        d[0] = make_uint4(p[pl][0], p[pl][1], p[pl][2], p[pl][3]);
+        d[1] = make_uint4(p[pl][4], p[pl][5], p[pl][6], p[pl][7]);
+      }
+    }
+  }
+}
+
+template <int Ci>
 __global__ void __launch_bounds__(512) gather2_kernel(Gather2Args a) {
-  extern __shared__ uint16_t sm_planes[];
   const GatherArgs& g = a.g;
   const int b = blockIdx.x, which = blockIdx.y, tid = threadIdx.x;
-  const int Ci = a.Ci, HW = g.H * g.W, npx = HW * Ci;
+  const int HW = g.H * g.W, npx = HW * Ci;
   const int Ec = npx + 4;
   long long slot = b;
   if (g.indices) slot = g.indices[b];
@@ -44,28 +100,7 @@
   const double clip_obs = g.normc[1];
   const bool norm_obs = g.normc[3] != 0.0;
   const float scale = g.scale;
-  const int rowe = g.W * Ci, pitch = rowe + 8, plane_e = g.H * pitch;
-  for (int e4 = tid; e4 < (npx >> 2); e4 += blockDim.x) {
-    const float4 v = frame_load4(src, g.fmt, npx, Ci, 4 * e4);
-    float y[4] = {v.x, v.y, v.z, v.w};
-    if (norm_obs) {
-      const double2 m0 = *reinterpret_cast<const double2*>(g.mean + 4 * e4), m1 = *reinterpret_cast<const double2*>(g.mean + 4 * e4 + 2);
-      const double2 i0 = *reinterpret_cast<const double2*>(g.var + 4 * e4), i1 = *reinterpret_cast<const double2*>(g.var + 4 * e4 + 2);
-      y[0] = (float)fmin(fmax(((double)y[0] - m0.x) * i0.x, -clip_obs), clip_obs);
-      y[1] = (float)fmin(fmax(((double)y[1] - m0.y) * i0.y, -clip_obs), clip_obs);
-      y[2] = (float)fmin(fmax(((double)y[2] - m1.x) * i1.x, -clip_obs), clip_obs);
-      y[3] = (float)fmin(fmax(((double)y[3] - m1.y) * i1.y, -clip_obs), clip_obs);
-    }
-    uint16_t p[3][4];
-#pragma unroll
-    for (int j = 0; j < 4; ++j) split3(y[j] / scale, p[0][j], p[1][j], p[2][j]);
-#pragma unroll
-    for (int pl = 0; pl < 3; ++pl) {
-      const uint2 w = make_uint2((uint32_t)p[pl][0] | ((uint32_t)p[pl][1] << 16), (uint32_t)p[pl][2] | ((uint32_t)p[pl][3] << 16));
-      const int e = 4 * e4, row = e / rowe, col = e - row * rowe;
-      *reinterpret_cast<uint2*>(sm_planes + pl * plane_e + row * pitch + col) = w;
-    }
-  }
+  for (int it = tid; it < 512; it += blockDim.x) s2d_half_block<Ci>(a, src, it, which, b);
   if (tid == 0) {
     float yy = frame_elem(src, g.fmt, npx, Ci, npx);
     if (norm_obs) yy = (float)fmin(fmax(((double)yy - g.mean[npx]) * g.var[npx], -clip_obs), clip_obs);
@@ -80,23 +115,6 @@
       a.fp[1][0][po] = p0; a.fp[1][1][po] = p1; a.fp[1][2][po] = p2;
     }
   }
-  __syncthreads();
-  const int seg = 8 * Ci;
-  const int K1 = 64 * Ci, nruns = a.OH * a.OW * 8;
-  const size_t img = (size_t)b * a.OH * a.OW * K1;
-  for (int i = tid; i < nruns * (seg / 8); i += blockDim.x) {
-    const int part = i % (seg / 8), run = i / (seg / 8);
-    const int ky = run & 7, patch = run >> 3;
-    const int oy = patch / a.OW, ox = patch - oy * a.OW;
-    const int so = (4 * oy + ky) * pitch + 4 * ox * Ci + 8 * part;
-    const size_t go = img + (size_t)patch * K1 + ky * seg + 8 * part;
-#pragma unroll
-    for (int pl = 0; pl < 3; ++pl) {
-      const uint16_t* sp = sm_planes + pl * plane_e + so;
-      const uint2 lo = *reinterpret_cast<const uint2*>(sp), hi = *reinterpret_cast<const uint2*>(sp + 4);
-      *reinterpret_cast<uint4*>(a.a1[which][pl] + go) = make_uint4(lo.x, lo.y, hi.x, hi.y);
-    }
-  }
   if (which == 0 && g.act) {
     const int feat_dim = g.feat_col + 1;
     if (tid < g.n_act) {
@@ -122,6 +140,7 @@
   int R, N, np;
   int transpose;
   int ld, off0;
+  int k1_ci;
   int tile_start;
 };
 
@@ -167,7 +186,9 @@
       const size_t o = (size_t)(n + job.off0) * job.ld + rb;
       for (int k = 0; k < job.np; ++k) {
         uint16_t* d = job.dst[k] + o;
-        if (rb + 7 < job.R && (o & 7) == 0)
+        if (job.k1_ci) {
+          for (int u = 0; u < 8; ++u) if (rb + u < job.R) d[conv1_krow(rb + u, job.k1_ci) - rb] = p[k][u];
+        } else if (rb + 7 < job.R && (o & 7) == 0)
           *reinterpret_cast<uint4*>(d) = make_uint4((uint32_t)p[k][0] | ((uint32_t)p[k][1] << 16), (uint32_t)p[k][2] | ((uint32_t)p[k][3] << 16),
                                                     (uint32_t)p[k][4] | ((uint32_t)p[k][5] << 16), (uint32_t)p[k][6] | ((uint32_t)p[k][7] << 16));
         else
@@ -178,7 +199,7 @@
 }
 
 int add_maps(V2State& v, uint16_t* const* planes, int np, int rank, std::initializer_list<uint64_t> dims, std::initializer_list<uint64_t> strides_b,
-             std::initializer_list<uint32_t> box, std::initializer_list<uint32_t> estr = {}, bool allow_whole = true) {
+             std::initializer_list<uint32_t> box, std::initializer_list<uint32_t> estr = {}, bool allow_whole = true, int swizzle = 128) {
   uint64_t d[5] = {1, 1, 1, 1, 1}, s[5] = {0, 0, 0, 0, 0};
   uint32_t bx[5] = {1, 1, 1, 1, 1}, es[5] = {1, 1, 1, 1, 1};
   int i = 0; for (auto x : dims) d[i++] = x;
@@ -196,7 +217,7 @@
   if (pitch <= 0 || pitch % 16) return -1;
   d[rank] = (uint64_t)np; s[rank - 1] = (uint64_t)pitch; bx[rank] = whole ? (uint32_t)np : 1u; es[rank] = 1;
   CUtensorMap m;
-  if (cg_encode_map(&m, planes[0], rank + 1, d, s, bx, es) != 0) return -1;
+  if (cg_encode_map(&m, planes[0], rank + 1, d, s, bx, es, swizzle) != 0) return -1;
   v.maps.push_back(m);
   v.map_whole.push_back(whole ? 1 : 0);
   v.map_box_bytes.push_back((int)box_bytes);
@@ -222,7 +243,8 @@
   P.a_off = 0; P.a_pstride = 128 * 128;
   P.b_off = planes * P.a_pstride; P.b_pstride = n_tile * 128;
   P.tx_bytes = planes * (a_box_rows * 128 + n_tile * 128);
-  P.mn_major = 0; P.ksteps = 4; P.a_kstep = P.b_kstep = 32;
+  P.mn_major = 0; P.ksteps = 4; P.a_kstep = P.b_kstep = 32; P.a_kstep2 = 64;
+  P.a_desc = P.b_desc = cg_desc_bits(128, false, 0); P.a_moff = 64 * 128;
   P.umma_n = n_tile;
   P.nprod = planes == 3 ? 6 : (planes == 2 ? 3 : 1);
   P.d0 = 1 << 20; P.d1 = 1;
@@ -241,8 +263,9 @@
   P.a_off = 0; P.a_pstride = atom;
   P.b_off = 2 * planes * atom; P.b_pstride = b_atoms * atom;
   P.tx_bytes = planes * (a_atoms + b_atoms) * atom;
-  P.mn_major = 1; P.ksteps = kr / 16; P.a_kstep = P.b_kstep = 2048;
+  P.mn_major = 1; P.ksteps = kr / 16; P.a_kstep = P.b_kstep = 2048; P.a_kstep2 = 4096;
   P.a_lbo = planes * atom; P.b_lbo = atom;
+  P.a_desc = cg_desc_bits(128, true, P.a_lbo); P.b_desc = cg_desc_bits(128, true, P.b_lbo); P.a_moff = P.a_lbo;
   P.umma_n = 64 * b_atoms;
   P.nprod = planes == 3 ? 6 : (planes == 2 ? 3 : 1);
   P.d0 = 1 << 20; P.d1 = 1;
@@ -260,6 +283,8 @@
     if (P.planes * P.umma_n > 256) return b2g_fail(B2G_EINVAL, std::string("engine v2: planes x tile width exceeds one accumulator buffer (group ") + name + ")");
     if (!cg_shape_supported(P.umma_n, P.nprod, P.mn_major != 0, P.ksteps))
       return b2g_fail(B2G_EINVAL, std::string("engine v2: no cg_kernel instance for the tile shape of a problem in group ") + name);
+    if (P.tm_sub > 1 && !cg_epi_handoff(P.epi))
+      return b2g_fail(B2G_EINVAL, std::string("engine v2: a banded problem must have an ACT or DGRAD epilogue (group ") + name + ")");
     g.flops += 2.0 * P.tiles_m * 128.0 * P.tiles_n * P.umma_n * P.chunks * 64.0;
   }
   list.push_back(g);
@@ -324,20 +349,20 @@
 
 int v2_alloc(b2g_sac* h) {
   V2State& v = h->v2;
-  const int B = h->B, Ci = h->Cimg, K1 = 64 * Ci, KF = v.KF;
-  const size_t n1 = (size_t)B * 225 * 32, n2 = (size_t)B * 36 * 64, n3 = (size_t)B * 1024, na = (size_t)B * 225 * K1, nf = (size_t)B * KF;
-  uint16_t *bH1, *bH2, *bH3, *bF, *bA1;
+  const int B = h->B, Cp = s2d_channels(h->Cimg), K1 = 64 * Cp, KF = v.KF;
+  const size_t n1 = (size_t)B * 225 * 32, n2 = (size_t)B * 36 * 64, n3 = (size_t)B * 1024, ns = (size_t)B * 4096 * Cp, nf = (size_t)B * KF;
+  uint16_t *bH1, *bH2, *bH3, *bF, *bS;
   if (int rc = dev_alloc(h->allocs, h->stream, &bH1, 9 * n1)) return rc;
   if (int rc = dev_alloc(h->allocs, h->stream, &bH2, 9 * n2)) return rc;
   if (int rc = dev_alloc(h->allocs, h->stream, &bH3, 9 * n3)) return rc;
   if (int rc = dev_alloc(h->allocs, h->stream, &bF, 9 * nf)) return rc;
-  if (int rc = dev_alloc(h->allocs, h->stream, &bA1, 6 * na)) return rc;
+  if (int rc = dev_alloc(h->allocs, h->stream, &bS, 6 * ns)) return rc;
   for (int n = 0; n < 3; ++n)
     for (int p = 0; p < 3; ++p) {
       v.H1[n][p] = bH1 + (n * 3 + p) * n1; v.H2[n][p] = bH2 + (n * 3 + p) * n2; v.H3[n][p] = bH3 + (n * 3 + p) * n3;
       v.F[n][p] = bF + (n * 3 + p) * nf;
     }
-  for (int w = 0; w < 2; ++w) for (int p = 0; p < 3; ++p) v.A1[w][p] = bA1 + (w * 3 + p) * na;
+  for (int w = 0; w < 2; ++w) for (int p = 0; p < 3; ++p) v.S[w][p] = bS + (w * 3 + p) * ns;
   if (int rc = dev_alloc(h->allocs, h->stream, &v.z0v, (size_t)B * 3 * h->H)) return rc;
   auto palloc = [&](uint16_t** arr, int np, size_t count) -> int {
     const size_t pitch = (count + 63) / 64 * 64;
@@ -372,7 +397,7 @@
 int v2_create(b2g_sac* h) {
   V2State& v = h->v2;
   g_mk_state = &v;
-  const int B = h->B, Ci = h->Cimg, K1 = 64 * Ci, KF = v.KF, FS = h->FS, H = h->H;
+  const int B = h->B, Ci = h->Cimg, Cp = s2d_channels(Ci), K1 = 64 * Cp, KF = v.KF, FS = h->FS, H = h->H;
   const size_t n1 = (size_t)B * 225 * 32;
   const char* nets[3] = {"model/pi", "model/values_fn", "target/values_fn"};
   std::vector<Plane2Job> jobs;
@@ -384,9 +409,12 @@
     start += ((R + 63) / 64) * ((N + 31) / 32);
     jobs.push_back(j);
   };
-  add_job(h->p("model/pi/cnn1/w"), K1, 32, v.W1T[0], 3, 1, K1, 0);
-  add_job(h->p("model/values_fn/cnn1/w"), K1, 32, v.W1T[0], 3, 1, K1, 32);
-  add_job(h->p("target/values_fn/cnn1/w"), K1, 32, v.W1T[1], 3, 1, K1, 0);
+  add_job(h->p("model/pi/cnn1/w"), 64 * Ci, 32, v.W1T[0], 3, 1, K1, 0);
+  jobs.back().k1_ci = Ci;
+  add_job(h->p("model/values_fn/cnn1/w"), 64 * Ci, 32, v.W1T[0], 3, 1, K1, 32);
+  jobs.back().k1_ci = Ci;
+  add_job(h->p("target/values_fn/cnn1/w"), 64 * Ci, 32, v.W1T[1], 3, 1, K1, 0);
+  jobs.back().k1_ci = Ci;
   for (int n = 0; n < 3; ++n) {
     add_job(h->p(std::string(nets[n]) + "/cnn2/w"), 512, 64, v.W2T[n], 3, 1, 512, 0);
     add_job(h->p(std::string(nets[n]) + "/cnn3/w"), 576, 64, v.W3T[n], 3, 1, 576, 0);
@@ -428,16 +456,31 @@
     CgGroup g;
     for (int w = 0; w < 2; ++w) {
       const int N = w == 0 ? 64 : 32;
-      const int mA = add_maps(v, v.A1[w], NP, 2, {(uint64_t)K1, (uint64_t)B * 225}, {(uint64_t)K1 * 2}, {64, 128});
+      const int mA = Cp == 1 ? add_maps(v, v.S[w], NP, 3, {32, 15, (uint64_t)B * 16}, {32, 512}, {32, 16, 8}, {}, true, 64)
+                             : add_maps(v, v.S[w], NP, 3, {64, 16, (uint64_t)B * 16}, {128, 2048}, {64, 16, 8});
       const int mB = add_maps(v, v.W1T[w], NP, 2, {(uint64_t)K1, (uint64_t)N}, {(uint64_t)K1 * 2}, {64, (uint32_t)N});
       if (mA < 0 || mB < 0) return b2g_fail(B2G_ECUDA, "engine v2: cuTensorMapEncodeTiled failed (conv1)");
-      CgProblem P = kmajor(NP, N, Ci, Ci, 128);
-      P.nloads = 2;
-      P.ld[0] = mk_load(mA, 2, 0); P.ld[0].d_tm[1] = 128; P.ld[0].d_c2[0] = 64;
-      P.ld[1] = mk_load(mB, 2, P.b_off); P.ld[1].d_c2[0] = 64;
-      P.tiles_m = (B * 225 + 127) / 128;
-      P.epi = CG_EPI_ACT; P.rows_tile = 128; P.lim_rows = B * 225;
-      P.o_tm = 128 * 32; P.o0 = 32; P.n_valid = N; P.out_planes = 3;
+      CgProblem P;
+      if (Cp == 1) {
+        P = kmajor(NP, N, 1, 1, 128);
+        P.a_pstride = 128 * 64; P.a_kstep = 32; P.a_kstep2 = NP * P.a_pstride;
+        P.b_off = 2 * P.a_kstep2;
+        P.tx_bytes = NP * (2 * 128 * 64 + N * 128);
+        P.a_desc = cg_desc_bits(64, false, 0); P.a_moff = 64 * 64;
+        P.nloads = 3;
+        for (int a = 0; a < 2; ++a) { P.ld[a] = mk_load(mA, 3, a * P.a_kstep2); P.ld[a].c0[2] = a; P.ld[a].d_tm[2] = 8; }
+        P.ld[2] = mk_load(mB, 2, P.b_off);
+      } else {
+        P = kmajor(NP, N, 4, 2, 128);
+        P.nloads = 2;
+        P.ld[0] = mk_load(mA, 3, 0); P.ld[0].d_tm[2] = 8; P.ld[0].d_c1[2] = 1; P.ld[0].d_c2[1] = 1;
+        P.ld[1] = mk_load(mB, 2, P.b_off); P.ld[1].d_c1[0] = 128; P.ld[1].d_c2[0] = 64;
+      }
+      P.tiles_m = 2 * B;
+      P.epi = CG_EPI_ACT; P.rows_tile = 128; P.lim_rows = 2 * B * 128;
+      P.d0 = 16; P.d1 = 8; P.o0 = 32; P.o1 = 15 * 32; P.o_tm = 225 * 32;
+      P.tm_sub = 2; P.o_sub = 8 * 15 * 32; P.lim_i0 = 15; P.lim_i1 = 15;
+      P.n_valid = N; P.out_planes = 3;
       P.grp_stride = (int)h1_net;
       const int net0 = w == 0 ? 0 : 2;
       for (int p = 0; p < 3; ++p) P.out_p[p] = v.H1[net0][p];
@@ -695,16 +738,38 @@
       g.host[g.n++] = P;
     }
     {
-      const int mA = add_maps(v, v.A1[0], NB, 2, {(uint64_t)K1, (uint64_t)B * 225}, {(uint64_t)K1 * 2}, {64, 64});
-      const int mB = add_maps(v, v.dZ1, NB, 2, {64, (uint64_t)B * 225}, {128}, {64, 64});
+      const int mA = Cp == 1 ? add_maps(v, v.S[0], NB, 3, {32, 15, (uint64_t)B * 16}, {32, 512}, {32, 16, 4}, {}, true, 64)
+                             : add_maps(v, v.S[0], NB, 3, {64, 16, (uint64_t)B * 16}, {128, 2048}, {64, 16, 4});
+      const int mB = add_maps(v, v.dZ1, NB, 4, {64, 15, 15, (uint64_t)B}, {128, 15 * 128, 225 * 128}, {64, 16, 4, 1});
       if (mA < 0 || mB < 0) return b2g_fail(B2G_ECUDA, "engine v2: cuTensorMapEncodeTiled failed (conv1 wgrad)");
-      CgProblem P = mnmajor(NB, 64, 2, 1, (B * 225 + 63) / 64);
-      P.nloads = 3;
-      for (int a = 0; a < 2; ++a) { P.ld[a] = mk_load(mA, 2, a * P.a_lbo); P.ld[a].c0[0] = 64 * a; P.ld[a].d_tm[0] = 128; P.ld[a].d_c2[1] = 64; }
-      P.ld[2] = mk_load(mB, 2, P.b_off); P.ld[2].d_c2[1] = 64;
-      P.tiles_m = (K1 + 127) / 128; P.tiles_n = 1;
+      CgProblem P = mnmajor(NB, 64, 2, 1, 4 * B);
+      P.n2 = 4;
+      if (Cp == 1) {
+        P.a_pstride = 64 * 64; P.a_lbo = NB * P.a_pstride;
+        P.b_off = 2 * P.a_lbo;
+        P.tx_bytes = NB * (2 * 64 * 64 + 64 * 128);
+        P.a_kstep = 16 * 64; P.a_kstep2 = 2 * P.a_kstep; P.a_desc = cg_desc_bits(64, true, P.a_lbo); P.a_moff = 0;
+        P.nloads = 3;
+        for (int a = 0; a < 2; ++a) { P.ld[a] = mk_load(mA, 3, a * P.a_lbo); P.ld[a].c0[2] = a; P.ld[a].d_c1[2] = 16; P.ld[a].d_c2[2] = 4; }
+        P.tiles_m = 1;
+        P.d0 = 4; P.d1 = 4; P.o0 = 32; P.o1 = 8 * 32;
+        P.rgrp_rows = 16;
+        for (int l = 0; l < 4; ++l) P.rgrp_off[l] = (32 * (l >> 1) + 4 * (l & 1)) * 32;
+      } else {
+        for (int l = 0; l < 2; ++l) {
+          P.ld[l] = mk_load(mA, 3, l * P.a_lbo); P.ld[l].c0[1] = l; P.ld[l].d_tm[2] = 1; P.ld[l].d_c1[2] = 16; P.ld[l].d_c2[2] = 4;
+        }
+        P.nloads = 3;
+        P.tiles_m = 2;
+        P.d0 = 4; P.d1 = 4; P.o0 = 32; P.o1 = Ci * 32; P.o_tm = 32 * Ci * 32;
+        P.lim_i0 = Ci;
+        P.rgrp_rows = 16;
+        for (int j = 0; j < 8; ++j) P.rgrp_off[j] = (8 * Ci * (j & 3) + 4 * Ci * (j >> 2)) * 32;
+      }
+      P.ld[P.nloads - 1] = mk_load(mB, 4, P.b_off); P.ld[P.nloads - 1].d_c1[3] = 1; P.ld[P.nloads - 1].d_c2[2] = 4;
+      P.tiles_n = 1;
       P.splits = std::max(1, std::min(P.chunks, std::max(84 / P.tiles_m, (P.chunks + 15) / 16)));
-      P.lim_rows = K1; P.o_tm = 128 * 32; P.o0 = 32; P.n_valid = 64;
+      P.lim_rows = 64 * Cp; P.n_valid = 64;
       P.out_f = h->g("model/pi/cnn1/w"); P.f_grp = (long long)(h->g("model/values_fn/cnn1/w") - h->g("model/pi/cnn1/w")); P.atomic = 1;
       g.host[g.n++] = P;
     }
@@ -716,7 +781,7 @@
     for (auto& g : v.fwd) parts.push_back(&g);
     std::vector<Wire> w;
     for (int n = 0; n < 3; ++n) {
-      w.push_back({1, n, 0, n < 2 ? 0 : 1, 3 * 225, 128, 0});
+      w.push_back({1, n, 0, n < 2 ? 0 : 1, 6, 1, 0});
       w.push_back({2, n, 1, n, 8 * 36, 108, 0});
       w.push_back({3, n, 2, n, 128 * 16, 128, 0});
       w.push_back({4, n, 3, n, 128, 128, 0});
@@ -735,8 +800,8 @@
       w.push_back({3, n, 2, 2 * n, 72, 108, 0});
       w.push_back({4, n, 2, 2 * n, 144, 108, 1});
     }
-    w.push_back({4, 2, 3, 0, 64, 450, 1});
-    w.push_back({4, 2, 3, 1, 64, 450, 1});
+    w.push_back({4, 2, 3, 0, 1, 8, 1});
+    w.push_back({4, 2, 3, 1, 1, 8, 1});
     if (int rc = fuse_groups(h, parts, w, "bwd_fused", v.bwd_fused, n_ctr)) return rc;
     std::vector<const CgGroup*> pa(parts.begin(), parts.begin() + 2), pb(parts.begin() + 2, parts.end());
     std::vector<Wire> wa, wb;
@@ -746,8 +811,8 @@
       wb.push_back({1, n, 0, 2 * n, 72, 108, 0});
       wb.push_back({2, n, 0, 2 * n, 144, 108, 1});
     }
-    wb.push_back({2, 2, 1, 0, 64, 450, 1});
-    wb.push_back({2, 2, 1, 1, 64, 450, 1});
+    wb.push_back({2, 2, 1, 0, 1, 8, 1});
+    wb.push_back({2, 2, 1, 1, 1, 8, 1});
     if (int rc = fuse_groups(h, pa, wa, "bwd_fused_fc", v.bwd_fused, n_ctr)) return rc;
     if (int rc = fuse_groups(h, pb, wb, "bwd_fused_conv", v.bwd_fused, n_ctr)) return rc;
   }
@@ -772,16 +837,16 @@
   Gather2Args a{};
   a.g = ga;
   for (int w = 0; w < 2; ++w)
-    for (int p = 0; p < 3; ++p) a.a1[w][p] = v.A1[w][p];
+    for (int p = 0; p < 3; ++p) a.s1[w][p] = v.S[w][p];
   for (int n = 0; n < 3; ++n) for (int p = 0; p < 3; ++p) a.fp[n][p] = v.F[n][p];
-  a.KF = v.KF; a.Ci = h->Cimg; a.OH = h->H1; a.OW = h->W1;
-  const size_t smem = (size_t)3 * h->Hi * (h->Wi * h->Cimg + 8) * sizeof(uint16_t);
-  static size_t attr = 0;
-  if (smem > attr) {
-    CK(cudaFuncSetAttribute(gather2_kernel, cudaFuncAttributeMaxDynamicSharedMemorySize, (int)smem));
-    attr = smem;
-  }
-  gather2_kernel<<<dim3(ga.B, ga.next_obs || ga.next_frame ? 2 : 1), 512, smem, s>>>(a);
+  a.KF = v.KF;
+  const dim3 grid(ga.B, ga.next_obs || ga.next_frame ? 2 : 1);
+  switch (h->Cimg) {
+    case 1: gather2_kernel<1><<<grid, 512, 0, s>>>(a); break;
+    case 2: gather2_kernel<2><<<grid, 512, 0, s>>>(a); break;
+    case 3: gather2_kernel<3><<<grid, 512, 0, s>>>(a); break;
+    default: gather2_kernel<4><<<grid, 512, 0, s>>>(a); break;
+  }
   return 0;
 }
 
diff --git a/deep-rl-grasping_b200/csrc/sac.cu b/deep-rl-grasping_b200/csrc/sac.cu
--- a/deep-rl-grasping_b200/csrc/sac.cu
+++ b/deep-rl-grasping_b200/csrc/sac.cu
@@ -1050,7 +1050,7 @@
   DA(h->metrics, MET_COUNT); DA(h->counters, 8); DA(h->step_consts, 4); DA(h->d_lr, 1);
   const int64_t cap = cfg->buffer_capacity;
   {
-    h->v2.on = h->cnn && cfg->precision == B2G_PREC_BF16X3 && h->Hi == 64 && h->Wi == 64;
+    h->v2.on = h->cnn && cfg->precision == B2G_PREC_BF16X3 && h->Hi == 64 && h->Wi == 64 && h->Cimg <= 4;
     if (const char* dbg = getenv("B2G_CG_DEBUG")) h->v2.dbg = atoi(dbg);
   }
   {
diff --git a/deep-rl-grasping_b200/csrc/sac_internal.cuh b/deep-rl-grasping_b200/csrc/sac_internal.cuh
--- a/deep-rl-grasping_b200/csrc/sac_internal.cuh
+++ b/deep-rl-grasping_b200/csrc/sac_internal.cuh
@@ -23,10 +23,15 @@
 };
 
 
+__host__ __device__ constexpr int s2d_channels(int Ci) { return Ci == 1 ? 1 : 4; }
+__host__ __device__ inline int conv1_krow(int r, int Ci) {
+  const int ci = r % Ci, kx = (r / Ci) % 8, ky = r / (8 * Ci);
+  return ((((ky >> 2) * 2 + (kx >> 2)) * 4 + (ky & 3)) * 4 + (kx & 3)) * s2d_channels(Ci) + ci;
+}
 struct V2State {
   bool on = false;
   int KF = 576;
-  uint16_t* A1[2][3]{};
+  uint16_t* S[2][3]{};
   uint16_t* H1[3][3]{};
   uint16_t* H2[3][3]{};
   uint16_t* H3[3][3]{};
```

After: 2323 (median of 6 runs). 3.6% higher.
